# dell-research-harvard/effocr

Hardware: AMD Instinct MI355X
Metric: glyph-crops/sec end-to-end (encode+kNN), 224x224 bs=1024 (higher is better)
Workload: dtype bf16; 1 GPU; BASELINE configs[1]: vit_small_patch16_224 encoder (bf16 MFMA operands, fp32 accumulate/residual/LN/softmax), 1024x3x224x224 fp32 crops per GPU resident in HBM, 10000-row fp32 IndexFlatIP, k=10; seeded random-init weights; crops_per_gpu=1024, global_batch=1024, index_rows=10000, k=10, parallelism=1024 crops per GPU, weights+index replicated

## Files before the change

effocr_amd/_lib.py:

```python
import ctypes
import os
import subprocess
import threading

_HERE = os.path.dirname(os.path.abspath(__file__))
_CSRC = os.path.join(_HERE, "csrc")
SO_PATH = os.environ.get("EFFOCR_HIP_LIB") or os.path.join(_HERE, "libeffocr_hip.so")
SO_PATH_AB = os.path.join(_HERE, "libeffocr_hip_ab.so")

ABI_VERSION = 9
PREC = {"bf16": 0, "fp16": 1, "fp32": 2}
EPI = {"bias": 0, "bias_gelu": 1, "bias_resid": 2}

_lock = threading.Lock()
_lib = None
_loaded = {}


class EffOCRHipError(RuntimeError):
    pass


def build(force=False, verbose=False, ab=True):
    so = os.path.join(_HERE, "libeffocr_hip.so")
# ... 16 lines not shown
        SO_PATH = path or os.environ.get("EFFOCR_HIP_LIB") or os.path.join(_HERE, "libeffocr_hip.so")
        if SO_PATH != prev:
            _lib = _loaded.get(SO_PATH)
            if _lib is not None:
                EXPORTS = sorted(_declare(_lib).keys())
    return prev


def _declare(lib):
    c = ctypes
    vp, i32, i64, sz, f32p, i64p = c.c_void_p, c.c_int, c.c_int64, c.c_size_t, c.c_void_p, c.c_void_p
    sig = {
        "effocr_abi_version": (i32, []),
        "effocr_last_error": (c.c_char_p, []),
        "effocr_encoder_create": (i32, [c.c_char_p, i32, i32, c.POINTER(vp)]),
        "effocr_encoder_destroy": (None, [vp]),
        "effocr_encoder_embed_dim": (i32, [vp]),
        "effocr_encoder_num_params": (i32, [vp]),
        "effocr_encoder_param_name": (c.c_char_p, [vp, i32]),
        "effocr_encoder_param_numel": (i64, [vp, i32]),
        "effocr_encoder_set_param": (i32, [vp, c.c_char_p, vp, i64]),
        "effocr_encoder_weights_bytes": (sz, [vp]),
        "effocr_encoder_upload": (i32, [vp, vp, sz]),
        "effocr_encoder_workspace_bytes": (sz, [vp, i32]),
        "effocr_encoder_forward": (i32, [vp, f32p, i32, f32p, i32, vp, sz, vp]),
        "effocr_encoder_forward_ex": (i32, [vp, vp, i32, i32, f32p, i32, vp, sz, vp]),
        "effocr_encoder_check_status": (i32, [vp, vp, vp]),
        "effocr_encoder_reset_status": (i32, [vp, vp, vp]),
        "effocr_clock_sample": (i32, [vp, vp]),
        "effocr_encoder_set_chunk": (i32, [vp, i32]),
        "effocr_encoder_set_option": (i32, [vp, c.c_char_p, i32]),
        "effocr_op_ln_linear": (i32, [i32, i32, f32p, f32p, f32p, c.c_float, vp, f32p, f32p, vp, i32, i32, i32, vp]),
        "effocr_encoder_profile_begin": (i32, [vp, i32, c.c_char_p]),
        "effocr_encoder_profile_collect": (i32, [vp]),
        "effocr_encoder_profile_get": (i32, [vp, i32, c.POINTER(c.c_char_p), c.POINTER(c.c_double), c.POINTER(i32),
                                             c.POINTER(c.c_double)]),
        "effocr_encoder_profile_clock": (i32, [vp, i32, c.POINTER(c.c_double)]),
        "effocr_knn_workspace_bytes": (sz, [i64, i64, i32, i32]),
        "effocr_knn_ip_topk": (i32, [f32p, i64, f32p, i64, i32, i32, f32p, i64p, vp, sz, vp]),
        "effocr_knn_screen_workspace_bytes": (sz, [i64, i64, i32, i32]),
        "effocr_knn_set_option": (i32, [c.c_char_p, i32]),
        "effocr_knn_screen_flag_offset": (sz, [i64, i64, i32, i32]),
        "effocr_knn_ip_topk_screened": (i32, [f32p, i64, f32p, vp, i64, i32, i32, c.c_float, f32p, i64p, vp, sz, vp]),
        "effocr_convert_bf16": (i32, [f32p, i64, vp, vp]),
        "effocr_bf16_blocked_bytes": (sz, [i64, i32]),
        "effocr_convert_bf16_blocked": (i32, [f32p, i64, i32, vp, vp]),
        "effocr_knn_ip_topk_screened2": (i32, [f32p, i64, f32p, vp, vp, i64, i32, i32, c.c_float, f32p, i64p, vp, sz, vp]),
        "effocr_l2_normalize": (i32, [f32p, i64, i32, f32p, vp]),
        "effocr_gather_rows": (i32, [f32p, i64p, i64, i32, f32p, vp]),
        "effocr_crop_transform": (i32, [vp, i32, i32, i64, vp, i32, i32, i32, c.POINTER(c.c_float), c.POINTER(c.c_float),
                                        c.POINTER(c.c_float), f32p, vp]),
        "effocr_crop_transform_batch": (i32, [vp, i32, i64, i32, i32, i64, vp, i64, i32, i32, c.POINTER(c.c_float), c.POINTER(c.c_float),
                                              c.POINTER(c.c_float), f32p, vp]),
        "effocr_crop_transform_batch_ex": (i32, [vp, i32, i64, i32, i32, i64, vp, i64, i32, i32, c.POINTER(c.c_float), c.POINTER(c.c_float),
                                                 c.POINTER(c.c_float), i32, vp, vp]),
        "effocr_localizer_create": (i32, [c.c_char_p, i32, i32, i32, c.POINTER(vp)]),
        "effocr_localizer_destroy": (None, [vp]),
        "effocr_localizer_num_params": (i32, [vp]),
        "effocr_localizer_param_name": (c.c_char_p, [vp, i32]),
        "effocr_localizer_param_numel": (i64, [vp, i32]),
        "effocr_localizer_set_param": (i32, [vp, c.c_char_p, vp, i64]),
        "effocr_localizer_weights_bytes": (sz, [vp]),
        "effocr_localizer_upload": (i32, [vp, vp, sz]),
        "effocr_localizer_set_option": (i32, [vp, c.c_char_p, i32]),
        "effocr_localizer_num_predictions": (i64, [vp]),
        "effocr_localizer_num_outputs": (i32, [vp]),
        "effocr_localizer_workspace_bytes": (sz, [vp, i32]),
        "effocr_localizer_forward": (i32, [vp, f32p, i32, f32p, vp, sz, vp]),
        "effocr_letterbox": (i32, [vp, i32, i32, i64, i32, i32, i32, i32, i32, i32, i32, f32p, vp]),
        "effocr_nms_workspace_bytes": (sz, [i32, i32]),
        "effocr_nms_batch_workspace_bytes": (sz, [i32, i32, i32]),
        "effocr_nms": (i32, [f32p, i32, i32, c.c_float, c.c_float, i32, i32, c.c_float, i32, f32p, vp, vp, sz, vp]),
        "effocr_nms_batch": (i32, [f32p, i32, i32, i32, c.c_float, c.c_float, i32, i32, c.c_float, i32, f32p, vp, vp, sz, vp]),
        "effocr_parse_char_boxes": (i32, [f32p, vp, i32, i32, i32, i32, i32, i32, f32p, vp, vp, vp, vp]),
        "effocr_op_linear": (i32, [i32, i32, vp, vp, f32p, f32p, vp, i32, i32, i32, vp]),
        "effocr_op_layernorm": (i32, [i32, f32p, i64, i32, f32p, f32p, c.c_float, vp, vp]),
        "effocr_op_attention": (i32, [i32, vp, vp, i32, i32, i32, vp]),
        "effocr_op_linear_blocked": (i32, [i32, i32, vp, vp, f32p, f32p, vp, i32, i32, i32, i32, vp]),
        "effocr_op_mlp_blocked": (i32, [i32, f32p, f32p, f32p, c.c_float, vp, f32p, vp, f32p, f32p, i32, i32, i32, i32, vp, sz, vp]),
        "effocr_op_mlp_ln_blocked": (i32, [i32, f32p, f32p, f32p, c.c_float, vp, f32p, vp, f32p, f32p, f32p, f32p, vp, i32, i32, i32, i32, vp, sz, vp]),
        "effocr_op_proj_mlp_blocked": (i32, [i32, f32p, vp, vp, f32p, f32p, f32p, c.c_float, vp, f32p, vp, f32p, f32p, i32, i32, i32, i32, vp, sz, vp]),
        "effocr_op_qkv_attn_blocked": (i32, [i32, vp, vp, f32p, vp, i32, i32, i32, i32, vp]),
        "effocr_op_layernorm_blocked": (i32, [i32, f32p, i64, i32, f32p, f32p, c.c_float, vp, vp]),
    }
    for name, (res, args) in sig.items():
        if os.environ.get("EFFOCR_HIP_LIB") and not hasattr(lib, name):
            def _absent(*a, _n=name, **k):
                raise EffOCRHipError(f"{_n} is not exported by the library EFFOCR_HIP_LIB points at")
            setattr(lib, name, _absent)
            continue
        fn = getattr(lib, name)
        fn.restype = res
        fn.argtypes = args
    return sig


EXPORTS = None


def lib():
    global _lib, EXPORTS
    with _lock:
        if _lib is None:
            if not os.path.exists(SO_PATH):
                raise EffOCRHipError(
                    f"{SO_PATH} not found: the HIP extension is required (no CPU fallback). "
                    "Run `python -c 'import __graft_entry__ as g; g.build()'` or `make -C effocr_amd/csrc`.")
            handle = ctypes.CDLL(SO_PATH)
            EXPORTS = sorted(_declare(handle).keys())
            got = handle.effocr_abi_version()
            older_ok = bool(os.environ.get("EFFOCR_HIP_LIB")) and os.environ.get("EFFOCR_HIP_ALLOW_OLDER_ABI") == "1" and 0 < got <= ABI_VERSION
            if got != ABI_VERSION and not older_ok:
                raise EffOCRHipError(f"libeffocr_hip.so ABI version {got} != {ABI_VERSION} expected by this package: rebuild (make -C effocr_amd/csrc)")
            _lib = _loaded[SO_PATH] = handle
    return _lib


_family = {}


def _load_family(so_path, prefix, abi_version, signatures, label):
    with _lock:
        handle = _family.get(prefix)
        if handle is None:
            if not os.path.exists(so_path):
                raise EffOCRHipError(f"{so_path} not found: the {label} library is required (no CPU fallback). "
                                     "Run `python -c 'import __graft_entry__ as g; g.build()'` or `make -C effocr_amd/csrc`.")
            handle = ctypes.CDLL(so_path)
            for name, (res, args) in signatures.items():
                fn = getattr(handle, name)
                fn.restype, fn.argtypes = res, args
            got = getattr(handle, f"effocr_{prefix}_abi_version")()
            if got != abi_version:
                raise EffOCRHipError(f"{os.path.basename(so_path)} ABI version {got} != {abi_version} expected by this package: rebuild "
                                     "(make -C effocr_amd/csrc)")
            _family[prefix] = handle
    return handle


def _family_check(prefix):
    def check(rc, what=""):
        if rc != 0:
            msg = getattr(globals()[f"{prefix}_lib"](), f"effocr_{prefix}_last_error")()
            raise EffOCRHipError(f"{what} failed (code {rc}): {msg.decode() if msg else '?'}")
    check.__name__ = f"{prefix}_check"
    return check


HEAD_SO_PATH = os.path.join(_HERE, "libeffocr_head.so")
HEAD_ABI_VERSION = 1
HEAD_EXPORTS = ("effocr_head_abi_version", "effocr_head_last_error", "effocr_classifier_head_workspace_bytes",
                "effocr_classifier_head")


def _head_signatures():
    c = ctypes
    return {
        "effocr_head_abi_version": (c.c_int, []),
        "effocr_head_last_error": (c.c_char_p, []),
        "effocr_classifier_head_workspace_bytes": (c.c_size_t, [c.c_int64, c.c_int]),
        "effocr_classifier_head": (c.c_int, [c.c_void_p, c.c_int64, c.c_int, c.c_void_p, c.c_void_p, c.c_int, c.c_void_p,
                                             c.c_void_p, c.c_void_p, c.c_size_t, c.c_void_p]),
    }


def head_lib():
# ... 336 lines not shown
```

effocr_amd/csrc/api.hip:

```cpp
#include "../../include/effocr_hip.h"
#include "enc_core.hpp"


#include <math.h>
#include <algorithm>
#include <string.h>
#include <map>
#include <memory>
#include <string>
#include <vector>

namespace effocr {

namespace {

struct Param { std::string name; std::vector<int64_t> shape; int64_t numel; std::vector<float> data; bool set; };

struct VitCfg { int D, depth, heads, mlp; };
struct VitLayerOff { size_t ln1w, ln1b, qkvb, projb, ln2w, ln2b, fc1b, fc2b, qkvw, projw, fc1w, fc2w;
                     size_t qkvw_b, projw_b, fc1w_b, fc2w_b, projw_pp, fc2w_pp, projb_p, fc2b_p, qkvw_bv, qkvb_v;
                     size_t qkvw_bf, qkv_s, qkv_c, fc1w_bf, fc1_s, fc1_c; };
struct ConvSpec { std::string w, bn; int cin, cout, k, stride, pad; size_t w_off, b_off; };
struct CnxBlockOff { size_t dww, dwb, lnw, lnb, w1, b1, w2, b2, gamma; };
struct CnxStageOff { int C, Cp, depth; size_t dslnw, dslnb, dsw, dsb; std::vector<CnxBlockOff> blocks; };

}
}

using namespace effocr;

struct effocr_encoder {
  std::string arch;
  bool is_vit = false;
  int img = 224, prec = PREC_BF16, D = 0;
  std::vector<Param> params;
  std::map<std::string, int> index;
  VitCfg vit{};
  int T = 0, P = 0;
  size_t off_clspos0 = 0, off_pos = 0, off_patchb = 0, off_normw = 0, off_normb = 0, off_patchw = 0, off_patchw_b = 0;
  std::vector<VitLayerOff> layers;
  std::vector<ConvSpec> convs;
  bool is_cnx = false;
  std::vector<CnxStageOff> cnx;
  size_t cnx_stemw = 0, cnx_stemb = 0, cnx_stemlnw = 0, cnx_stemlnb = 0, cnx_headw = 0, cnx_headb = 0;
  bool is_mnv = false;
  MnvNet mnv{};
  size_t wbytes = 0;
  const char* wdev = nullptr;
  int debug = 0;
  int cls_only_last = 1;
  int mlp_stagger_min_rounds = 2;
  int mlp_tail_first = 96;
  int mlp_stagger = 2500;
  int use_projf = 1;
  int use_qkvattn = 1;
  int qa_min_batch = 1;
  int qa_hsplit = 0;
  int use_patchf = 1;
  int use_mlp = 1;
  int use_gemm3 = 1;
  int use_lnfold = 1;
  int tail_split = 1;
  int split6 = 1;
  int pair_parts = 1;
  int mlp_pair = 0;
  int use_blocked = 1;
  int use_gemm2 = 1;
  int panel_rows = 128;
  int use_panel = 1;
  int chunk = 0;
  int call_size_invariant = 0;
  int prof_mode = 0;
  std::string prof_only;
  std::vector<std::pair<hipEvent_t, hipEvent_t>> prof_pool;
  std::vector<std::pair<int, int>> prof_rec;
  std::vector<std::string> prof_names;
  size_t prof_used = 0;
  std::vector<float> prof_ms;
  std::vector<int> prof_cnt;
  std::vector<double> prof_work;
  unsigned long long* prof_clk = nullptr;
  std::vector<double> prof_ghz;
  static constexpr size_t PROF_CLK_SLOTS = 256;
};

namespace effocr {
namespace {

int64_t prod(const std::vector<int64_t>& s) { int64_t p = 1; for (auto v : s) p *= v; return p; }

void add_param(effocr_encoder* e, const std::string& name, std::vector<int64_t> shape) {
  Param p; p.name = name; p.shape = shape; p.numel = prod(shape); p.set = false;
  e->index[name] = (int)e->params.size();
  e->params.push_back(std::move(p));
}

void build_vit(effocr_encoder* e) {
  const int D = e->vit.D, depth = e->vit.depth, mlp = e->vit.mlp;
  e->P = (e->img / 16) * (e->img / 16);
  e->T = e->P + 1;
  add_param(e, "cls_token", {1, 1, D});
  add_param(e, "pos_embed", {1, e->T, D});
  add_param(e, "patch_embed.proj.weight", {D, 3, 16, 16});
  add_param(e, "patch_embed.proj.bias", {D});
  for (int i = 0; i < depth; ++i) {
    const std::string p = "blocks." + std::to_string(i) + ".";
    add_param(e, p + "norm1.weight", {D});
    add_param(e, p + "norm1.bias", {D});
    add_param(e, p + "attn.qkv.weight", {3 * D, D});
    add_param(e, p + "attn.qkv.bias", {3 * D});
    add_param(e, p + "attn.proj.weight", {D, D});
    add_param(e, p + "attn.proj.bias", {D});
    add_param(e, p + "norm2.weight", {D});
    add_param(e, p + "norm2.bias", {D});
    add_param(e, p + "mlp.fc1.weight", {mlp, D});
    add_param(e, p + "mlp.fc1.bias", {mlp});
    add_param(e, p + "mlp.fc2.weight", {D, mlp});
    add_param(e, p + "mlp.fc2.bias", {D});
  }
  add_param(e, "norm.weight", {D});
  add_param(e, "norm.bias", {D});

  const size_t es = prec_esize(e->prec);
  Alloc a;
  e->off_clspos0 = a.take((size_t)D * 4);
  e->off_pos = a.take((size_t)e->T * D * 4);
  e->off_patchb = a.take((size_t)D * 4);
  e->layers.resize(depth);
  for (int i = 0; i < depth; ++i) {
    VitLayerOff& L = e->layers[i];
    L.ln1w = a.take((size_t)D * 4); L.ln1b = a.take((size_t)D * 4);
    L.qkvb = a.take((size_t)3 * D * 4); L.projb = a.take((size_t)D * 4);
    L.ln2w = a.take((size_t)D * 4); L.ln2b = a.take((size_t)D * 4);
// ... 396 lines not shown
      put_pw(b.pwl, p + ".conv_pwl.weight", p + ".bn3");
    }
    if (r.se) { put_plain(b.ser, p + ".se.conv_reduce"); put_plain(b.see, p + ".se.conv_expand"); }
  }
  put_pw(n.cn, "blocks.5.0.conv.weight", "blocks.5.0.bn1");
  const auto& hw = P(e, "conv_head.weight"); const auto& hb = P(e, "conv_head.bias");
  put_op(blob, n.head.w, hw.data(), hw.size(), e->prec); put_f32(blob, n.head.b, hb.data(), hb.size());
}

int prof_class(effocr_encoder* e, const char* name) {
  for (size_t i = 0; i < e->prof_names.size(); ++i) if (e->prof_names[i] == name) return (int)i;
  e->prof_names.push_back(name);
  e->prof_work.push_back(0.0);
  return (int)e->prof_names.size() - 1;
}

template <typename F>
int timed(effocr_encoder* e, const char* name, double work, hipStream_t s, F launch) {
  const bool on = e->prof_mode == 1 || (e->prof_mode == 2 && e->prof_only == name);
  if (!on) return launch();
  if (e->prof_used == e->prof_pool.size()) {
    hipEvent_t a, b;
    if (hipEventCreate(&a) != hipSuccess || hipEventCreate(&b) != hipSuccess) return fail(EFFOCR_EHIP, "profile: hipEventCreate failed");
    e->prof_pool.push_back({a, b});
  }
  const int cls = prof_class(e, name);
  const size_t slot = e->prof_used++;
  const bool clk = e->prof_mode == 1 && slot < effocr_encoder::PROF_CLK_SLOTS &&
                   (e->prof_clk || hipMalloc(&e->prof_clk, effocr_encoder::PROF_CLK_SLOTS * 8192 * sizeof(unsigned long long)) == hipSuccess && hipMemset(e->prof_clk, 0, effocr_encoder::PROF_CLK_SLOTS * 8192 * sizeof(unsigned long long)) == hipSuccess);
  if (clk) (void)clock_sample(e->prof_clk + slot * 8192, s);
  (void)hipEventRecord(e->prof_pool[slot].first, s);
  const int rc = launch();
  (void)hipEventRecord(e->prof_pool[slot].second, s);
  if (clk) (void)clock_sample(e->prof_clk + slot * 8192 + 4096, s);
  e->prof_rec.push_back({cls, (int)slot});
  e->prof_work[cls] += work;
  return rc;
}

struct VitWs { size_t status, x, xn, qkv, att, h, stats, total, rows, hbytes; };
VitWs vit_ws(const effocr_encoder* e, int B) {
  const size_t M = align_up((size_t)B * e->T, 128), D = e->vit.D, es = prec_esize(e->prec);
  Alloc a; VitWs w;
  w.rows = M;
  w.status = a.take(256);
  w.x = a.take(M * D * 4);
  w.xn = a.take(M * D * es);
  w.qkv = a.take(M * 3 * D * es);
  w.att = a.take(M * D * es);
  size_t hb = M * e->vit.mlp * es, pb = (size_t)B * e->P * 768 * es;
  w.hbytes = hb > pb ? hb : pb;
  {
    const size_t cus = (size_t)device_cus(), np = M / 128, tail = np % cus;
    const size_t split = (tail && tail * 6 <= cus) ? 6 : (tail && tail * 4 <= cus) ? 4 : (tail && tail * 2 <= cus) ? 2 : 0;
    const size_t need = split * tail * 128 * D * 4;
    if (need > w.hbytes) w.hbytes = need;
  }
  w.h = a.take(w.hbytes);
  w.stats = a.take(M * 64);
  w.total = a.off;
  return w;
}

int vit_forward(effocr_encoder* e, const void* x, int x16, int B, float* emb, int l2, char* ws, hipStream_t s) {
  const VitWs w = vit_ws(e, B);
  const int D = e->vit.D, T = e->T, Pn = e->P, M = B * T, prec = e->prec;
  const char* wb = e->wdev;
  float* xs = reinterpret_cast<float*>(ws + w.x);
  void* xn = ws + w.xn; void* qkv = ws + w.qkv; void* att = ws + w.att; void* hb = ws + w.h;
  auto F = [&](size_t off) { return reinterpret_cast<const float*>(wb + off); };
  int rc;
  const double Md = (double)M, Dd = (double)D, Hd = (double)e->vit.mlp;
  const bool panel = e->use_panel && panel_gemm_supported(prec, 3 * D, D) && panel_gemm_supported(prec, e->vit.mlp, D);
  const bool g2 = e->use_gemm2 && gemm2_supported(prec, D, e->vit.mlp);
  const bool g2p = e->use_gemm2 && gemm2_supported(prec, D, 768);
  const bool g3all = !panel && e->use_gemm3 && gemm3_supported(prec, 3 * D, D) && gemm3_supported(prec, D, D) &&
                     gemm3_supported(prec, e->vit.mlp, D) && gemm3_supported(prec, D, e->vit.mlp);
  const int blk = (e->use_blocked && g2p && ((panel && g2) || g3all)) ? 1 : 0;
  const bool mlpf = blk && panel && e->use_mlp && mlp_fused_supported(prec, D, e->vit.mlp);
  const bool projf = mlpf && e->use_projf;
  const bool qaf = blk && panel && mlpf && qkv_attn_supported(prec, D, T) && (e->use_qkvattn == 2 || (e->use_qkvattn == 1 && (e->call_size_invariant || B >= e->qa_min_batch)));
  const bool g3 = blk && e->use_gemm3 && gemm3_supported(prec, D, e->vit.mlp);
  const bool patchf = blk && e->use_patchf && patch_embed_fused_supported(prec, D);
  if (!patchf && (rc = timed(e, "im2col_patch16", 0.0, s, [&] { return im2col_patch16(prec, x, x16, B, e->img, e->img, hb, s); }))) return rc;
  int* status = reinterpret_cast<int*>(ws + w.status);
  if (!patchf && (rc = set_cls_rows(F(e->off_clspos0), xs, B, T, D, blk, nullptr, s))) return rc;
  GemmArgs g{};
  if (patchf) {
    PatchArgs pa{};
    pa.x = x; pa.x16 = x16; pa.B = B; pa.H = e->img; pa.W = e->img; pa.Wb = wb + e->off_patchw_b; pa.bias = F(e->off_patchb); pa.pos = F(e->off_pos);
    pa.out = xs; pa.D = D; pa.P = Pn; pa.cls = F(e->off_clspos0);
    if ((rc = timed(e, "patch_embed_fused", 2.0 * B * Pn * Dd * 768.0, s, [&] { return patch_embed_fused(prec, pa, s); }))) return rc;
  } else {
  g.X = hb; g.ldx = 768; g.W = wb + e->off_patchw; g.ldw = 768; g.bias = F(e->off_patchb);
  g.out = xs; g.ldo = D; g.pos = F(e->off_pos); g.M = B * Pn; g.N = D; g.K = 768; g.P = Pn; g.blk_out = blk;
  if ((rc = timed(e, "gemm_patch_embed", 2.0 * B * Pn * Dd * 768.0, s, [&] { return g2p ? gemm2_nt(prec, EPI_PATCH, g, s) : gemm_nt(prec, EPI_PATCH, g, s); }))) return rc;
  }
  const float* cls_x = nullptr;
  bool xn_ready = false;
  for (int i = 0; i < e->vit.depth; ++i) {
    const VitLayerOff& L = e->layers[i];
    if (panel) {
      {
      PanelArgs p{};
      if (qaf) {
        if (!xn_ready && (rc = timed(e, "layernorm", 0.0, s, [&] { return layernorm_rows_blocked(prec, xs, M, D, F(L.ln1w), F(L.ln1b), 1e-6f, xn, s); }))) return rc;
        xn_ready = false;
        QkvAttnArgs q{};
        q.xn = xn; q.Wb = wb + L.qkvw_bv; q.bias = F(L.qkvb_v); q.out = att;
        q.B = B; q.T = T; q.D = D; q.rows_alloc = (int64_t)w.rows; q.hsplit = e->qa_hsplit;
        q.cls_only = (i + 1 == e->vit.depth && e->cls_only_last && projf) ? 1 : 0;
        const bool cls_k = q.cls_only && D == 384 && T > 192;
        const double qa_work = cls_k ? 2.0 * Md * 2.0 * Dd * Dd + 2.0 * (32.0 * B) * Dd * Dd + 4.0 * B * e->vit.heads * 32.0 * T * 64.0
                                     : 2.0 * Md * 3.0 * Dd * Dd + 4.0 * B * e->vit.heads * (double)T * T * 64.0;
        if ((rc = timed(e, "qkv_attn_fused", qa_work, s, [&] { return qkv_attn_fused(prec, q, s); }))) return rc;
      } else {
      p.A = xs; p.lda = D; p.gamma = F(L.ln1w); p.beta = F(L.ln1b); p.eps = 1e-6f; p.W = wb + L.qkvw; p.bias = F(L.qkvb);
      p.out = qkv; p.ldo = 3 * D; p.M = M; p.N = 3 * D; p.K = D; p.rows_padded = 1; p.debug = e->debug; p.panel_rows = e->panel_rows; p.no_tail_split = !e->tail_split;
      p.blk_a = blk; p.blk_out = blk;
      if ((rc = timed(e, "panel_ln_qkv", 2.0 * Md * 3.0 * Dd * Dd, s, [&] { return panel_gemm(prec, PRO_LN, EPI_BIAS, p, s); }))) return rc;
      if ((rc = timed(e, "attention", 4.0 * B * e->vit.heads * (double)T * T * 64.0, s, [&] { return attention(prec, qkv, att, B, T, e->vit.heads, blk, s); }))) return rc;
      }
      if (!projf) {
      p = PanelArgs{};
      p.A = att; p.lda = D; p.W = wb + L.projw; p.bias = F(L.projb); p.out = xs; p.ldo = D; p.resid = xs; p.ldr = D;
      p.M = M; p.N = D; p.K = D; p.rows_padded = 1; p.debug = e->debug; p.panel_rows = e->panel_rows; p.no_tail_split = !e->tail_split; p.blk_a = blk; p.blk_out = blk;
      if ((rc = timed(e, "panel_proj_resid", 2.0 * Md * Dd * Dd, s, [&] { return panel_gemm(prec, PRO_COPY, EPI_BIAS_RESID, p, s); }))) return rc;
      }
      }
      if (mlpf) {
        MlpArgs m{};
        m.x = xs; m.gamma = F(L.ln2w); m.beta = F(L.ln2b); m.eps = 1e-6f; m.W1b = wb + L.fc1w_b; m.b1 = F(L.fc1b);
        m.W2p = wb + L.fc2w_pp; m.b2 = F(L.fc2b_p); m.b2_logical = F(L.fc2b); m.M = M; m.D = D; m.H = e->vit.mlp; m.rows_alloc = (int)w.rows;
        m.partial = reinterpret_cast<float*>(hb); m.partial_bytes = w.hbytes; m.no_tail_split = !e->tail_split; m.no_split6 = !e->split6; m.pair = e->mlp_pair; m.no_pair_parts = !e->pair_parts; m.stagger = e->mlp_stagger; m.stagger_min_rounds = e->mlp_stagger_min_rounds; m.tail_first = e->mlp_tail_first;
        if (e->call_size_invariant) { m.no_tail_split = 1; m.pair = -1; }
        if (projf) {
          m.A = att; m.Wpp = wb + L.projw_pp; m.bp = F(L.projb_p);
          if (i + 1 == e->vit.depth && e->cls_only_last) {
            const size_t Bp = align_up((size_t)B, 128);
            float* xc = reinterpret_cast<float*>(qkv);
            void* ac = static_cast<char*>(qkv) + Bp * D * 4;
            if ((rc = timed(e, "gather_cls", 0.0, s, [&] { return gather_cls_rows_blocked(xs, att, B, T, D, xc, ac, s); }))) return rc;
            m.x = xc; m.A = ac; m.M = B; m.rows_alloc = (int)Bp;
            const double Bd = B;
            if ((rc = timed(e, "proj_mlp_cls", 4.0 * Bd * Hd * Dd + 2.0 * Bd * Dd * Dd, s, [&] { return mlp_fused(prec, m, s); }))) return rc;
            cls_x = xc;
            continue;
          }
          if (qaf && i + 1 < e->vit.depth) {
            m.xn_out = xn; m.gamma_n = F(e->layers[i + 1].ln1w); m.beta_n = F(e->layers[i + 1].ln1b);
            xn_ready = true;
          }
          if ((rc = timed(e, "proj_mlp_fused", 4.0 * Md * Hd * Dd + 2.0 * Md * Dd * Dd, s, [&] { return mlp_fused(prec, m, s); }))) return rc;
          continue;
        }
        if (qaf && i + 1 < e->vit.depth) {
          m.xn_out = xn; m.gamma_n = F(e->layers[i + 1].ln1w); m.beta_n = F(e->layers[i + 1].ln1b);
          xn_ready = true;
        }
        if ((rc = timed(e, "mlp_fused", 4.0 * Md * Hd * Dd, s, [&] { return mlp_fused(prec, m, s); }))) return rc;
        continue;
      }
      PanelArgs p{};
      p.A = xs; p.lda = D; p.gamma = F(L.ln2w); p.beta = F(L.ln2b); p.eps = 1e-6f; p.W = wb + L.fc1w; p.bias = F(L.fc1b);
      p.out = hb; p.ldo = e->vit.mlp; p.M = M; p.N = e->vit.mlp; p.K = D; p.rows_padded = 1; p.debug = e->debug; p.panel_rows = e->panel_rows; p.no_tail_split = !e->tail_split;
      p.blk_a = blk; p.blk_out = blk;
      if ((rc = timed(e, "panel_ln_fc1_gelu", 2.0 * Md * Hd * Dd, s, [&] { return panel_gemm(prec, PRO_LN, EPI_BIAS_GELU, p, s); }))) return rc;
    } else if (blk) {
      const bool fold = e->use_lnfold && g3 && gemm3_lnfold_supported(D);
      float* stats = reinterpret_cast<float*>(ws + w.stats);
      auto lin = [&](const void* X, int K, size_t wblk, const float* bias, void* out, int N, int epi, int fl = 0, const float* cs = nullptr) {
        GemmArgs q{};
        q.X = X; q.ldx = K; q.Wblk = wb + wblk; q.bias = bias; q.out = out; q.ldo = N; q.M = M; q.N = N; q.K = K;
        q.blk_x = 1; q.blk_out = 1; q.rows_alloc = (int)w.rows; q.no_tail_split = !e->tail_split;
        if (epi == EPI_BIAS_RESID) { q.resid = xs; q.ldr = N; }
        if (fl == 1) { q.lnf = 1; q.lnf_stats = stats; q.lnf_s = cs; q.lnf_eps = 1e-6f; }
        if (fl == 2) { q.stats = stats; q.x16 = xn; }
        return gemm3_nt(prec, epi, q, s);
      };
      const bool fold1 = fold && i > 0;
      if (!fold1 && (rc = timed(e, "layernorm", 0.0, s, [&] { return layernorm_rows_blocked(prec, xs, M, D, F(L.ln1w), F(L.ln1b), 1e-6f, xn, s); }))) return rc;
      if ((rc = timed(e, "gemm_qkv", 2.0 * Md * 3.0 * Dd * Dd, s, [&] {
            return fold1 ? lin(xn, D, L.qkvw_bf, F(L.qkv_c), qkv, 3 * D, EPI_BIAS, 1, F(L.qkv_s)) : lin(xn, D, L.qkvw_b, F(L.qkvb), qkv, 3 * D, EPI_BIAS); }))) return rc;
      if ((rc = timed(e, "attention", 4.0 * B * e->vit.heads * (double)T * T * 64.0, s, [&] { return attention(prec, qkv, att, B, T, e->vit.heads, 1, s); }))) return rc;
      const size_t Bp = align_up((size_t)B, 256);
      if (i + 1 == e->vit.depth && e->cls_only_last && g3 && Bp <= w.rows) {
        float* xc = reinterpret_cast<float*>(qkv);
        void* ac = static_cast<char*>(qkv) + Bp * D * 4;
        if ((rc = timed(e, "gather_cls", 0.0, s, [&] { return gather_cls_rows_blocked(xs, att, B, T, D, xc, ac, s); }))) return rc;
        auto linc = [&](const void* X, int K, size_t wblk, const float* bias, void* out, int N, int epi, int fl = 0, const float* cs = nullptr) {
          GemmArgs q{};
          q.X = X; q.ldx = K; q.Wblk = wb + wblk; q.bias = bias; q.out = out; q.ldo = N; q.M = B; q.N = N; q.K = K;
          q.blk_x = 1; q.blk_out = 1; q.rows_alloc = (int)Bp; q.no_tail_split = !e->tail_split;
          if (epi == EPI_BIAS_RESID) { q.resid = xc; q.ldr = N; }
          if (fl == 1) { q.lnf = 1; q.lnf_stats = stats; q.lnf_s = cs; q.lnf_eps = 1e-6f; }
          if (fl == 2) { q.stats = stats; q.x16 = xn; }
          return gemm3_nt(prec, epi, q, s);
        };
        const double Bd = B;
        if ((rc = timed(e, "cls_proj_resid", 2.0 * Bd * Dd * Dd, s, [&] { return linc(ac, D, L.projw_b, F(L.projb), xc, D, EPI_BIAS_RESID, fold ? 2 : 0); }))) return rc;
        if (!fold && (rc = timed(e, "layernorm", 0.0, s, [&] { return layernorm_rows_blocked(prec, xc, B, D, F(L.ln2w), F(L.ln2b), 1e-6f, xn, s); }))) return rc;
        if ((rc = timed(e, "cls_fc1_gelu", 2.0 * Bd * Hd * Dd, s, [&] {
              return fold ? linc(xn, D, L.fc1w_bf, F(L.fc1_c), hb, e->vit.mlp, EPI_BIAS_GELU, 1, F(L.fc1_s)) : linc(xn, D, L.fc1w_b, F(L.fc1b), hb, e->vit.mlp, EPI_BIAS_GELU); }))) return rc;
        if ((rc = timed(e, "cls_fc2_resid", 2.0 * Bd * Dd * Hd, s, [&] { return linc(hb, e->vit.mlp, L.fc2w_b, F(L.fc2b), xc, D, EPI_BIAS_RESID); }))) return rc;
        cls_x = xc;
        continue;
      }
      if ((rc = timed(e, "gemm_proj_resid", 2.0 * Md * Dd * Dd, s, [&] { return lin(att, D, L.projw_b, F(L.projb), xs, D, EPI_BIAS_RESID, fold ? 2 : 0); }))) return rc;
      if (!fold && (rc = timed(e, "layernorm", 0.0, s, [&] { return layernorm_rows_blocked(prec, xs, M, D, F(L.ln2w), F(L.ln2b), 1e-6f, xn, s); }))) return rc;
      if ((rc = timed(e, "gemm_fc1_gelu", 2.0 * Md * Hd * Dd, s, [&] {
            return fold ? lin(xn, D, L.fc1w_bf, F(L.fc1_c), hb, e->vit.mlp, EPI_BIAS_GELU, 1, F(L.fc1_s)) : lin(xn, D, L.fc1w_b, F(L.fc1b), hb, e->vit.mlp, EPI_BIAS_GELU); }))) return rc;
      if (fold && g3 && i + 1 < e->vit.depth) {
        GemmArgs q{};
        q.X = hb; q.ldx = e->vit.mlp; q.Wblk = wb + L.fc2w_b; q.bias = F(L.fc2b); q.out = xs; q.ldo = D; q.resid = xs; q.ldr = D;
        q.M = M; q.N = D; q.K = e->vit.mlp; q.blk_x = 1; q.blk_out = 1; q.rows_alloc = (int)w.rows; q.no_tail_split = !e->tail_split;
        q.stats = stats; q.x16 = xn;
        if ((rc = timed(e, "gemm_fc2_resid", 2.0 * Md * Dd * Hd, s, [&] { return gemm3_nt(prec, EPI_BIAS_RESID, q, s); }))) return rc;
        continue;
      }
    } else {
      if ((rc = timed(e, "layernorm", 0.0, s, [&] { return layernorm_rows(prec, xs, M, D, F(L.ln1w), F(L.ln1b), 1e-6f, xn, s); }))) return rc;
      g = GemmArgs{};
      g.X = xn; g.ldx = D; g.W = wb + L.qkvw; g.ldw = D; g.bias = F(L.qkvb); g.out = qkv; g.ldo = 3 * D;
      g.M = M; g.N = 3 * D; g.K = D;
      if ((rc = timed(e, "gemm_qkv", 2.0 * Md * 3.0 * Dd * Dd, s, [&] { return gemm_nt(prec, EPI_BIAS, g, s); }))) return rc;
      if ((rc = timed(e, "attention", 4.0 * B * e->vit.heads * (double)T * T * 64.0, s, [&] { return attention(prec, qkv, att, B, T, e->vit.heads, 0, s); }))) return rc;
      g = GemmArgs{};
      g.X = att; g.ldx = D; g.W = wb + L.projw; g.ldw = D; g.bias = F(L.projb); g.out = xs; g.ldo = D;
      g.resid = xs; g.ldr = D; g.M = M; g.N = D; g.K = D;
      if ((rc = timed(e, "gemm_proj_resid", 2.0 * Md * Dd * Dd, s, [&] { return gemm_nt(prec, EPI_BIAS_RESID, g, s); }))) return rc;
      if ((rc = timed(e, "layernorm", 0.0, s, [&] { return layernorm_rows(prec, xs, M, D, F(L.ln2w), F(L.ln2b), 1e-6f, xn, s); }))) return rc;
      g = GemmArgs{};
      g.X = xn; g.ldx = D; g.W = wb + L.fc1w; g.ldw = D; g.bias = F(L.fc1b); g.out = hb; g.ldo = e->vit.mlp;
      g.M = M; g.N = e->vit.mlp; g.K = D;
// ... 245 lines not shown
    if (!(T <= 64 || (T > 192 && T <= 224)))
      return fail(EFFOCR_EUNSUPPORTED, "vit: token count must be <= 64 or in (192, 224] (img_size 224)");
    e->is_vit = true; e->D = e->vit.D;
    build_vit(e.get());
  }
  *out = e.release();
  return EFFOCR_OK;
}

void effocr_encoder_destroy(effocr_encoder_t* enc) {
  if (!enc) return;
  for (auto& ev : enc->prof_pool) { (void)hipEventDestroy(ev.first); (void)hipEventDestroy(ev.second); }
  if (enc->prof_clk) (void)hipFree(enc->prof_clk);
  delete enc;
}
int effocr_encoder_embed_dim(const effocr_encoder_t* enc) { return enc ? enc->D : 0; }
int effocr_encoder_num_params(const effocr_encoder_t* enc) { return enc ? (int)enc->params.size() : 0; }
const char* effocr_encoder_param_name(const effocr_encoder_t* enc, int i) {
  if (!enc || i < 0 || i >= (int)enc->params.size()) return nullptr;
  return enc->params[i].name.c_str();
}
int64_t effocr_encoder_param_numel(const effocr_encoder_t* enc, int i) {
  if (!enc || i < 0 || i >= (int)enc->params.size()) return -1;
  return enc->params[i].numel;
}

int effocr_encoder_set_param(effocr_encoder_t* enc, const char* name, const float* host, int64_t numel) {
  if (!enc || !name || !host) return fail(EFFOCR_EINVAL, "set_param: NULL argument");
  auto it = enc->index.find(name);
  if (it == enc->index.end()) return fail(EFFOCR_EINVAL, std::string("set_param: unknown parameter '") + name + "'");
  Param& p = enc->params[it->second];
  if (p.numel != numel)
    return fail(EFFOCR_EINVAL, std::string("set_param: '") + name + "' expects " + std::to_string(p.numel) +
                                   " elements, got " + std::to_string(numel));
  p.data.assign(host, host + numel);
  p.set = true;
  return EFFOCR_OK;
}

size_t effocr_encoder_weights_bytes(const effocr_encoder_t* enc) { return enc ? enc->wbytes : 0; }

int effocr_encoder_upload(effocr_encoder_t* enc, void* weights_dev, size_t bytes) {
  if (!enc || !weights_dev) return fail(EFFOCR_EINVAL, "upload: NULL argument");
  if (bytes < enc->wbytes) return fail(EFFOCR_EWORKSPACE, "upload: weight buffer too small");
  for (const Param& p : enc->params)
    if (!p.set) return fail(EFFOCR_ESTATE, "upload: parameter '" + p.name + "' was never set");
  std::vector<char> blob(enc->wbytes, 0);
  if (enc->is_vit) pack_vit(enc, blob); else if (enc->is_cnx) pack_convnext(enc, blob); else if (enc->is_mnv) pack_mobilenetv3(enc, blob);
  else pack_resnet(enc, blob);
  const hipError_t er = hipMemcpy(weights_dev, blob.data(), enc->wbytes, hipMemcpyHostToDevice);
  if (er != hipSuccess) return fail(EFFOCR_EHIP, std::string("upload: hipMemcpy: ") + hipGetErrorString(er));
  enc->wdev = static_cast<const char*>(weights_dev);
  return EFFOCR_OK;
}

size_t effocr_encoder_workspace_bytes(const effocr_encoder_t* enc, int batch) {
  if (!enc || batch <= 0) return 0;
  if (enc->is_cnx) return convnext_ws(enc, cnx_chunk(enc, batch)).total;
  if (enc->is_mnv) return mnv3_ws(enc, mnv3_chunk(enc, batch)).total;
  if (!enc->is_vit) return resnet_ws(enc, batch).total;
  return vit_ws(enc, (enc->chunk > 0 && enc->chunk < batch) ? enc->chunk : batch).total;
}

int effocr_encoder_set_option(effocr_encoder_t* enc, const char* name, int value) {
  if (!enc || !name) return fail(EFFOCR_EINVAL, "set_option: NULL argument");
  const std::string n = name;
  if (n == "use_panel") { enc->use_panel = value; return EFFOCR_OK; }
  if (n == "debug") { enc->debug = value; return EFFOCR_OK; }
  if (n == "use_gemm2") { enc->use_gemm2 = value; return EFFOCR_OK; }
  if (n == "use_blocked") { enc->use_blocked = value; return EFFOCR_OK; }
  if (n == "tail_split") { enc->tail_split = value; return EFFOCR_OK; }
  if (n == "split6") { enc->split6 = value; return EFFOCR_OK; }
  if (n == "mlp_pair") { enc->mlp_pair = value; return EFFOCR_OK; }
  if (n == "pair_parts") { enc->pair_parts = value; return EFFOCR_OK; }
  if (n == "use_gemm3") { enc->use_gemm3 = value; return EFFOCR_OK; }
  if (n == "use_lnfold") { enc->use_lnfold = value; return EFFOCR_OK; }
  if (n == "use_mlp") { enc->use_mlp = value; return EFFOCR_OK; }
  if (n == "use_qkvattn") { enc->use_qkvattn = value; return EFFOCR_OK; }
  if (n == "qa_min_batch") { enc->qa_min_batch = value; return EFFOCR_OK; }
  if (n == "qa_hsplit") { enc->qa_hsplit = value; return EFFOCR_OK; }
  if (n == "use_patchf") { enc->use_patchf = value; return EFFOCR_OK; }
  if (n == "use_projf") { enc->use_projf = value; return EFFOCR_OK; }
  if (n == "cls_only_last") { enc->cls_only_last = value; return EFFOCR_OK; }
  if (n == "mlp_stagger_min_rounds") { enc->mlp_stagger_min_rounds = value < 1 ? 1 : value; return EFFOCR_OK; }
  if (n == "mlp_tail_first") { enc->mlp_tail_first = value < 0 ? 0 : value & ~7; return EFFOCR_OK; }
  if (n == "mlp_stagger") { enc->mlp_stagger = value < 0 ? 0 : value; return EFFOCR_OK; }
  if (n == "panel_rows") { if (value != 64 && value != 128) return fail(EFFOCR_EINVAL, "set_option: panel_rows must be 64 or 128"); enc->panel_rows = value; return EFFOCR_OK; }
  if (n == "call_size_invariant") {
    if (value != 0 && value != 1) return fail(EFFOCR_EINVAL, "set_option: call_size_invariant must be 0 or 1");
    enc->call_size_invariant = value; return EFFOCR_OK;
  }
  if (n == "chunk") { if (value < 0) return fail(EFFOCR_EINVAL, "set_option: chunk < 0"); enc->chunk = value; return EFFOCR_OK; }
  return fail(EFFOCR_EINVAL, "set_option: unknown option '" + n + "'");
}

int effocr_encoder_set_chunk(effocr_encoder_t* enc, int crops_per_chunk) {
  if (!enc || crops_per_chunk < 0) return fail(EFFOCR_EINVAL, "set_chunk: bad argument");
  enc->chunk = crops_per_chunk;
  return EFFOCR_OK;
}

int effocr_encoder_forward(effocr_encoder_t* enc, const float* x_dev, int batch, float* emb_dev, int l2_normalize,
                           void* workspace_dev, size_t workspace_bytes, void* stream) {
  return effocr_encoder_forward_ex(enc, x_dev, EFFOCR_PREC_FP32, batch, emb_dev, l2_normalize, workspace_dev, workspace_bytes, stream);
}

int effocr_encoder_forward_ex(effocr_encoder_t* enc, const void* x_dev, int x_dtype, int batch, float* emb_dev, int l2_normalize,
                              void* workspace_dev, size_t workspace_bytes, void* stream) {
  if (!enc) return fail(EFFOCR_EINVAL, "forward: NULL encoder");
  if (x_dtype != PREC_FP32 && !(enc->is_vit && enc->prec != PREC_FP32 && x_dtype == enc->prec))
    return fail(x_dtype < 0 || x_dtype > 2 ? EFFOCR_EINVAL : EFFOCR_EUNSUPPORTED,
                "forward: crops must be fp32, or (ViT, 16-bit precision modes) already in the encoder's own operand type");
  const int x16 = x_dtype != PREC_FP32;
  if (batch < 0) return fail(EFFOCR_EINVAL, "forward: negative batch");
  if (batch == 0) return EFFOCR_OK;
  if (!x_dev || !emb_dev || !workspace_dev) return fail(EFFOCR_EINVAL, "forward: NULL device pointer");
  if (!enc->wdev) return fail(EFFOCR_ESTATE, "forward: weights were not uploaded");
  if (workspace_bytes < effocr_encoder_workspace_bytes(enc, batch)) return fail(EFFOCR_EWORKSPACE, "forward: workspace too small");
  if ((int64_t)batch * (enc->is_vit ? enc->T : enc->img * enc->img) >= (int64_t)1 << 30)
    return fail(EFFOCR_EUNSUPPORTED, "forward: batch too large for 32-bit row indices");
  char* ws = static_cast<char*>(workspace_dev);
  if (enc->is_cnx) {
    const int chunk = cnx_chunk(enc, batch);
    const int64_t so = enc->img / 4;
    if ((int64_t)chunk * so * so * 4 * enc->cnx[0].C >= (int64_t)1 << 31)
      return fail(EFFOCR_EUNSUPPORTED, "forward: chunk too large for 32-bit GEMM row indices (effocr_encoder_set_chunk)");
    const size_t img_bytes = (size_t)3 * enc->img * enc->img * 4;
    for (int b0 = 0; b0 < batch; b0 += chunk) {
      const int cb = (batch - b0 < chunk) ? batch - b0 : chunk;
      const int rc = convnext_forward(enc, reinterpret_cast<const float*>(static_cast<const char*>(x_dev) + (size_t)b0 * img_bytes), cb,
                                      emb_dev + (size_t)b0 * enc->D, l2_normalize, ws, S(stream));
      if (rc) return rc;
    }
    return EFFOCR_OK;
  }
  if (enc->is_mnv) {
    const int chunk = mnv3_chunk(enc, batch);
    const size_t img_bytes = (size_t)3 * enc->img * enc->img * 4;
    for (int b0 = 0; b0 < batch; b0 += chunk) {
      const int cb = (batch - b0 < chunk) ? batch - b0 : chunk;
      const int rc = mnv3_forward(enc, reinterpret_cast<const float*>(static_cast<const char*>(x_dev) + (size_t)b0 * img_bytes), cb,
                                  emb_dev + (size_t)b0 * enc->D, l2_normalize, ws, S(stream));
      if (rc) return rc;
    }
    return EFFOCR_OK;
  }
  if (!enc->is_vit) return resnet_forward(enc, static_cast<const float*>(x_dev), batch, emb_dev, l2_normalize, ws, S(stream));
  const int chunk = enc->chunk > 0 ? enc->chunk : batch;
  const size_t img_bytes = (size_t)3 * enc->img * enc->img * (x16 ? 2 : 4);
  for (int b0 = 0; b0 < batch; b0 += chunk) {
    const int cb = (batch - b0 < chunk) ? batch - b0 : chunk;
    const int rc = vit_forward(enc, static_cast<const char*>(x_dev) + (size_t)b0 * img_bytes, x16, cb, emb_dev + (size_t)b0 * enc->D, l2_normalize, ws, S(stream));
    if (rc) return rc;
  }
  return EFFOCR_OK;
}

int effocr_clock_sample(void* out_dev, void* stream) {
  if (!out_dev) return fail(EFFOCR_EINVAL, "clock_sample: NULL pointer");
  return clock_sample(static_cast<unsigned long long*>(out_dev), S(stream));
}

int effocr_encoder_check_status(const effocr_encoder_t* enc, const void* workspace_dev, void* stream) {
  if (!enc || !workspace_dev) return fail(EFFOCR_EINVAL, "check_status: NULL argument");
  if (!enc->is_vit && !enc->is_cnx && !enc->is_mnv) return EFFOCR_OK;
  int st = 0;
// ... 187 lines not shown
    p.A = x_dev; p.lda = k; p.W = w_dev; p.bias = bias_dev; p.out = out_dev; p.ldo = n; p.resid = resid_dev; p.ldr = n;
    p.M = m; p.N = n; p.K = k;
    return panel_gemm(precision, PRO_COPY, epilogue, p, S(stream));
  }
  GemmArgs g{};
  g.X = x_dev; g.ldx = k; g.W = w_dev; g.ldw = k; g.bias = bias_dev; g.out = out_dev; g.ldo = n;
  g.resid = resid_dev; g.ldr = n; g.M = m; g.N = n; g.K = k;
  if (gemm2_supported(precision, n, k)) return gemm2_nt(precision, epilogue, g, S(stream));
  return gemm_nt(precision, epilogue, g, S(stream));
}

int effocr_op_ln_linear(int precision, int epilogue, const float* x_dev, const float* gamma_dev, const float* beta_dev,
                        float eps, const void* w_dev, const float* bias_dev, const float* resid_dev, void* out_dev,
                        int m, int n, int k, void* stream) {
  if (epilogue < 0 || epilogue > 2) return fail(EFFOCR_EINVAL, "op_ln_linear: unknown epilogue");
  PanelArgs p{};
  p.A = x_dev; p.lda = k; p.gamma = gamma_dev; p.beta = beta_dev; p.eps = eps; p.W = w_dev; p.bias = bias_dev;
  p.out = out_dev; p.ldo = n; p.resid = resid_dev; p.ldr = n; p.M = m; p.N = n; p.K = k;
  return panel_gemm(precision, PRO_LN, epilogue, p, S(stream));
}


int effocr_op_linear_blocked(int precision, int epilogue, const void* x_blk_dev, const void* w_blk_dev, const float* bias_dev,
                             const float* resid_blk_dev, void* out_blk_dev, int m, int n, int k, int rows_alloc, void* stream) {
  if (epilogue < 0 || epilogue > 2) return fail(EFFOCR_EINVAL, "op_linear_blocked: unknown epilogue");
  if (m > 0 && (!x_blk_dev || !w_blk_dev || !bias_dev || !out_blk_dev || (epilogue == EPI_BIAS_RESID && !resid_blk_dev)))
    return fail(EFFOCR_EINVAL, "op_linear_blocked: NULL device pointer");
  GemmArgs g{};
  g.X = x_blk_dev; g.ldx = k; g.Wblk = w_blk_dev; g.bias = bias_dev; g.out = out_blk_dev; g.ldo = n;
  g.resid = resid_blk_dev; g.ldr = n; g.M = m; g.N = n; g.K = k; g.blk_x = 1; g.blk_out = 1; g.rows_alloc = rows_alloc;
  return gemm3_nt(precision, epilogue, g, S(stream));
}

int effocr_op_mlp_blocked(int precision, float* x_blk_dev, const float* gamma_dev, const float* beta_dev, float eps,
                          const void* w1_blk_dev, const float* b1_dev, const void* w2_perm_dev, const float* b2_perm_dev, const float* b2_dev,
                          int m, int d, int h, int rows_alloc, void* scratch_dev, size_t scratch_bytes, void* stream) {
  if (m > 0 && (!x_blk_dev || !gamma_dev || !beta_dev || !w1_blk_dev || !b1_dev || !w2_perm_dev || !b2_perm_dev || !b2_dev))
    return fail(EFFOCR_EINVAL, "op_mlp_blocked: NULL device pointer");
  MlpArgs a{};
  a.x = x_blk_dev; a.gamma = gamma_dev; a.beta = beta_dev; a.eps = eps; a.W1b = w1_blk_dev; a.b1 = b1_dev; a.W2p = w2_perm_dev; a.b2 = b2_perm_dev;
  a.b2_logical = b2_dev;
  a.M = m; a.D = d; a.H = h; a.rows_alloc = rows_alloc; a.partial = static_cast<float*>(scratch_dev); a.partial_bytes = scratch_bytes;
  return mlp_fused(precision, a, S(stream));
}

int effocr_op_mlp_ln_blocked(int precision, float* x_blk_dev, const float* gamma_dev, const float* beta_dev, float eps,
                             const void* w1_blk_dev, const float* b1_dev, const void* w2_perm_dev, const float* b2_perm_dev, const float* b2_dev,
                             const float* gamma_next_dev, const float* beta_next_dev, void* xn_blk_dev,
                             int m, int d, int h, int rows_alloc, void* scratch_dev, size_t scratch_bytes, void* stream) {
  if (m > 0 && (!x_blk_dev || !gamma_dev || !beta_dev || !w1_blk_dev || !b1_dev || !w2_perm_dev || !b2_perm_dev || !b2_dev || !gamma_next_dev || !beta_next_dev || !xn_blk_dev))
    return fail(EFFOCR_EINVAL, "op_mlp_ln_blocked: NULL device pointer");
  MlpArgs a{};
  a.x = x_blk_dev; a.gamma = gamma_dev; a.beta = beta_dev; a.eps = eps; a.W1b = w1_blk_dev; a.b1 = b1_dev; a.W2p = w2_perm_dev; a.b2 = b2_perm_dev;
  a.b2_logical = b2_dev;
  a.M = m; a.D = d; a.H = h; a.rows_alloc = rows_alloc; a.partial = static_cast<float*>(scratch_dev); a.partial_bytes = scratch_bytes;
  a.xn_out = xn_blk_dev; a.gamma_n = gamma_next_dev; a.beta_n = beta_next_dev;
  return mlp_fused(precision, a, S(stream));
}

int effocr_op_proj_mlp_blocked(int precision, float* x_blk_dev, const void* a_blk_dev, const void* wp_perm_dev, const float* bp_perm_dev,
                               const float* gamma_dev, const float* beta_dev, float eps, const void* w1_blk_dev, const float* b1_dev,
                               const void* w2_perm_dev, const float* b2_perm_dev, const float* b2_dev, int m, int d, int h, int rows_alloc,
                               void* scratch_dev, size_t scratch_bytes, void* stream) {
  if (m > 0 && (!x_blk_dev || !a_blk_dev || !wp_perm_dev || !bp_perm_dev || !gamma_dev || !beta_dev || !w1_blk_dev || !b1_dev || !w2_perm_dev || !b2_perm_dev || !b2_dev))
    return fail(EFFOCR_EINVAL, "op_proj_mlp_blocked: NULL device pointer");
  MlpArgs a{};
  a.x = x_blk_dev; a.gamma = gamma_dev; a.beta = beta_dev; a.eps = eps; a.W1b = w1_blk_dev; a.b1 = b1_dev; a.W2p = w2_perm_dev; a.b2 = b2_perm_dev;
  a.b2_logical = b2_dev; a.A = a_blk_dev; a.Wpp = wp_perm_dev; a.bp = bp_perm_dev;
  a.M = m; a.D = d; a.H = h; a.rows_alloc = rows_alloc; a.partial = static_cast<float*>(scratch_dev); a.partial_bytes = scratch_bytes;
  return mlp_fused(precision, a, S(stream));
}

int effocr_op_qkv_attn_blocked(int precision, const void* xn_blk_dev, const void* wqkv_blk_dev, const float* bias_dev,
                               void* out_blk_dev, int batch, int tokens, int d, int rows_alloc, void* stream) {
  if (batch > 0 && (!xn_blk_dev || !wqkv_blk_dev || !bias_dev || !out_blk_dev))
    return fail(EFFOCR_EINVAL, "op_qkv_attn_blocked: NULL device pointer");
  if (batch < 0 || tokens < 1) return fail(EFFOCR_EINVAL, "op_qkv_attn_blocked: bad batch / tokens");
  QkvAttnArgs q{};
  q.xn = xn_blk_dev; q.Wb = wqkv_blk_dev; q.bias = bias_dev; q.out = out_blk_dev;
  q.B = batch; q.T = tokens; q.D = d; q.rows_alloc = rows_alloc;
  return qkv_attn_fused(precision, q, S(stream));
}

int effocr_op_layernorm_blocked(int out_precision, const float* x_blk_dev, int64_t rows, int d, const float* gamma_dev,
                                const float* beta_dev, float eps, void* out_blk_dev, void* stream) {
  if (rows > 0 && (!x_blk_dev || !gamma_dev || !beta_dev || !out_blk_dev)) return fail(EFFOCR_EINVAL, "op_layernorm_blocked: NULL device pointer");
  return layernorm_rows_blocked(out_precision, x_blk_dev, rows, d, gamma_dev, beta_dev, eps, out_blk_dev, S(stream));
}

int effocr_op_layernorm(int out_precision, const float* x_dev, int64_t rows, int d, const float* gamma_dev,
                        const float* beta_dev, float eps, void* out_dev, void* stream) {
  return layernorm_rows(out_precision, x_dev, rows, d, gamma_dev, beta_dev, eps, out_dev, S(stream));
}

int effocr_op_attention(int precision, const void* qkv_dev, void* out_dev, int batch, int tokens, int heads, void* stream) {
  return attention(precision, qkv_dev, out_dev, batch, tokens, heads, 0, S(stream));
}

}
```

effocr_amd/csrc/kernels.hpp:

```cpp
#pragma once
#include "common.hpp"

namespace effocr {

enum { PREC_BF16 = 0, PREC_FP16 = 1, PREC_FP32 = 2 };
enum { EPI_BIAS = 0, EPI_BIAS_GELU = 1, EPI_BIAS_RESID = 2, EPI_PATCH = 3,
       EPI_BIAS_SCALE_RESID = 4,
       EPI_BIAS_F32 = 5 };

static inline int prec_esize(int prec) { return prec == PREC_FP32 ? 4 : 2; }

struct GemmArgs {
  const void* X; int64_t ldx;
  const void* W; int64_t ldw;
  const float* bias;
  void* out; int64_t ldo;
  const float* resid; int64_t ldr;
  const float* pos;
  int M, N, K;
  int P;
  int blk_x;
  int blk_out;
  const void* Wblk;
  int rows_alloc;
  int no_tail_split;
  float* stats; void* x16;
  const float* lnf_stats; const float* lnf_s; int lnf; float lnf_eps;
  const float* scale;
};

int gemm_nt(int prec, int epi, const GemmArgs& g, hipStream_t s);

bool gemm2_supported(int prec, int N, int K);
int gemm2_nt(int prec, int epi, const GemmArgs& g, hipStream_t s);

bool gemm3_supported(int prec, int N, int K);
bool gemm3_lnfold_supported(int D);
int gemm3_nt(int prec, int epi, const GemmArgs& g, hipStream_t s);

struct MlpArgs {
  float* x;
  const float* gamma; const float* beta; float eps;
  const void* W1b; const float* b1;
  const void* W2p; const float* b2;
  int M, D, H;
  int rows_alloc;
  float* partial; size_t partial_bytes;
  int no_tail_split;
  int no_split6;
  int no_pair_parts;
  int pair;
  int panel0, tail_rb, stagger_wgs, main_wgs;
  int stagger;
  int stagger_min_rounds;
  int tail_first;
  const void* A; const void* Wpp; const float* bp; const float* b2_logical;
  void* xn_out; const float* gamma_n; const float* beta_n;
};
bool mlp_fused_supported(int prec, int D, int H);
int mlp_fused(int prec, const MlpArgs& a, hipStream_t s);

struct QkvAttnArgs {
  const void* xn;
  const void* Wb; const float* bias;
  void* out;
  int B, T, D;
  int64_t rows_alloc;
  int cls_only;
  int img0;
  int hsplit;
};
bool qkv_attn_supported(int prec, int D, int T);
int qkv_attn_fused(int prec, const QkvAttnArgs& a, hipStream_t s);

struct PatchArgs {
  const void* x; int B, H, W;
  int x16;
  const void* Wb;
  const float* bias; const float* pos;
  const float* cls;
  float* out;
  int D, P;
};
bool patch_embed_fused_supported(int prec, int D);
int patch_embed_fused(int prec, const PatchArgs& a, hipStream_t s);

enum { PRO_COPY = 0, PRO_LN = 1 };
struct PanelArgs {
  const void* A; int64_t lda;
  const float* gamma; const float* beta; float eps;
  const void* W;
  const float* bias;
  void* out; int64_t ldo;
  const float* resid; int64_t ldr;
  int M, N, K;
  unsigned long long* dbg;
  int debug;
  int blk_a;
  int blk_out;
  int panel_rows;
  int rows_padded;
  int no_tail_split;
  int tail_first, tail_split;
};
bool panel_gemm_supported(int prec, int N, int K);
int panel_gemm(int prec, int pro, int epi, const PanelArgs& a, hipStream_t s);

int reduce_layernorm_rows_blocked(int prec_out, float* x, int64_t rows, int D, const float* partial, const float* b2, int nparts, int tail_rb,
                                  int add_x, const float* gamma, const float* beta, float eps, void* out, hipStream_t s);
int layernorm_rows_blocked(int prec_out, const float* x, int64_t rows, int D, const float* gamma, const float* beta,
                           float eps, void* out, hipStream_t s);
int layernorm_rows(int prec_out, const float* x, int64_t rows, int D, const float* gamma, const float* beta,
                   float eps, void* out, hipStream_t s);
int im2col_patch16(int prec_out, const void* x, int x16, int B, int H, int W, void* out, hipStream_t s);
int clock_sample(unsigned long long* out, hipStream_t s);
int set_cls_rows(const float* cls_pos0, float* x, int B, int T, int D, int blocked, int* status_zero, hipStream_t s);
int gather_cls_rows_blocked(const float* x, const void* att, int B, int T, int D, float* xc, void* ac, hipStream_t s);
int attention(int prec, const void* qkv, void* out, int B, int T, int heads, int blocked, hipStream_t s);
int final_cls_norm(const float* x, int B, int T, int D, const float* gamma, const float* beta, float eps,
                   int l2norm, int blocked, float* emb, int* status, hipStream_t s);

size_t knn_workspace_bytes(int64_t B, int64_t N, int D, int k);
int knn_ip_topk(const float* q, int64_t B, const float* xb, int64_t N, int D, int k, float* dist, int64_t* idx,
                void* ws, size_t ws_bytes, hipStream_t s);
size_t knn_screen_workspace_bytes(int64_t B, int64_t N, int D, int k);
void knn_set_wg_target(int n);
void knn_q16_tile(int on);
void knn_two_pass_screen(int on);
void knn_force_tile_kernel(int on);
size_t knn_screen_flag_offset(int64_t B, int64_t N, int D, int k);
int knn_ip_topk_screened(const float* q, int64_t B, const float* xb, const void* xb16, const void* xblk, int64_t N, int D, int k, float xnorm_max,
                         float* dist, int64_t* idx, void* ws, size_t ws_bytes, hipStream_t s);
int convert_bf16_blocked(const float* src, int64_t N, int D, void* dst, hipStream_t s);
void knn_qs_option(int which, int value);
int convert_bf16(const float* src, int64_t n, void* dst, hipStream_t s);
int l2_normalize_rows(const float* x, int64_t B, int D, float* y, hipStream_t s);
int gather_rows(const float* src, const int64_t* rows, int64_t n, int D, float* dst, hipStream_t s);

int crop_transform(const uint8_t* img, int n_img, int64_t img_stride, int H, int W, int64_t stride, const int* boxes, int box_ld, int64_t n, int S,
                   int antialias, const float* mean, const float* stdv, const float* fill, void* out, int out_prec, hipStream_t s);

struct ConvArgs {
  const float* in;
  const float* w;
  const float* bias;
  const float* resid;
  float* out;
  int B, H, W, Cin, Cout, KH, KW, stride, pad, OH, OW, relu;
  int in_ld, in_off, out_ld, out_off, res_ld, res_off;
  int silu;
  float* partial; size_t partial_bytes;
  int ksplit;
  const void* w16;
};
int conv2d_nhwc(const ConvArgs& a, hipStream_t s);
int im2col_conv1(const float* x, float* col, int B, int H, int W, int OH, int OW, hipStream_t s);
int maxpool3x3s2_nhwc(const float* in, float* out, int B, int H, int W, int C, int OH, int OW, hipStream_t s);
int global_avgpool_nhwc(const float* in, float* out, int B, int HW, int C, int l2norm, hipStream_t s);

int im2col_nchw(const float* x, float* col, int B, int Cin, int H, int W, int KH, int KW, int stride, int pad, int OH, int OW, int kpad, hipStream_t s);
int stem6x6s2_nchw(const float* x, const float* w, int w_ld, const float* wt, const float* bias, float* out, int B, int H, int W, int OH, int OW, int out_ld,
                   int out_off, int silu, hipStream_t s);
int stem6x6s2_g16_nchw(const float* x, const float* wt, int wt_ld, const float* bias, float* out, int B, int H, int W, int OH, int OW, int out_ld,
                       int out_off, int cout, int cout_st, hipStream_t s);
int upsample2x_nhwc(const float* in, int in_ld, int in_off, float* out, int out_ld, int out_off, int B, int H, int W, int C, hipStream_t s);
int maxpool5_nhwc(const float* in, int in_ld, int in_off, float* out, int out_ld, int out_off, int B, int H, int W, int C, hipStream_t s);
int yolo_decode(const float* raw, int raw_ld, float* pred, int B, int ny, int nx, int na, int no, float stride, const float* anchors_px,
                int64_t total, int64_t row0, hipStream_t s);
int letterbox_u8(const uint8_t* img, int H, int W, int64_t row_stride, int bgr, int out_h, int out_w, int new_h, int new_w, int top, int left,
                 float fill, float* out, hipStream_t s);
size_t nms_workspace_bytes(int n, int max_nms);
bool nms_greedy_applies(int n, int max_det, int max_nms);
int nms_yolo_batch(const float* pred, int B, int n, int nc, float conf_thres, float iou_thres, int max_det, int max_nms, float max_wh, int agnostic,
                   float* out, int* count, void* ws, size_t ws_bytes, hipStream_t s);
int nms_yolo(const float* pred, int n, int nc, float conf_thres, float iou_thres, int max_det, int max_nms, float max_wh, int agnostic,
             float* out, int* count, void* ws, size_t ws_bytes, hipStream_t s);

int stem3x3s2_nchw(const float* x, const float* wt, int wt_ld, const float* bias, float* out, int B, int H, int W, int OH, int OW, int out_ld, int out_off,
                   int cout, int cout_st, hipStream_t s);
int yolov8_decode(const float* box, int box_ld, const float* cls, int cls_ld, float* pred, int B, int ny, int nx, int nc, float stride, int64_t total,
                  int64_t row0, hipStream_t s);

constexpr int Y11_MAX_TOKENS = 1600;
int attention_nhwc(const float* qkv, int qkv_ld, int qkv_off, float* out, int out_ld, int out_off, int B, int N, int heads, hipStream_t s);
int dwconv3x3_nhwc(const float* in, int in_ld, int in_off, int icut, int istride, const float* w, const float* bias, int silu, const float* add, int add_ld,
                   int add_off, float* out, int out_ld, int out_off, int B, int H, int W, int C, hipStream_t s);

int cnx_stem(const float* img, int B, int S, const float* wt, const float* bias, const float* lnw, const float* lnb, int C0, float* x, hipStream_t s);
int cnx_dwconv_ln(int prec, const float* x, int B, int H, int W, int C, int Cp, const float* w, const float* bias, const float* lnw,
                  const float* lnb, void* out, hipStream_t s);
int cnx_ln_s2d(int prec, const float* x, int B, int H, int W, int C, int Cp, const float* lnw, const float* lnb, void* out, hipStream_t s);
int cnx_head(const float* x, int B, int HW, int C, int Cp, const float* lnw, const float* lnb, int l2norm, float* emb, int* status, hipStream_t s);

struct MnvConv { uint32_t w, b; };
struct MnvBlock { int cin, mid, cout, k, stride, se, hs, res, cg; MnvConv pw, dw, ser, see, pwl; };
constexpr int MNV_NBLK = 11;
struct MnvNet { int S, stem_c, cn_c, nf; MnvConv stem, cn, head; MnvBlock blk[MNV_NBLK]; };
constexpr int MNV_T1 = 8, MNV_T2 = 8;
constexpr int MNV_TAIL_LDS_FLOATS = 39680;
__host__ __device__ static inline int mnv3_tiles1(int S) { const int n = (S / 4 + MNV_T1 - 1) / MNV_T1; return n * n; }
__host__ __device__ static inline int mnv3_tiles2(int S) { const int n = (S / 8 + MNV_T2 - 1) / MNV_T2; return n * n; }
int mnv3_stem_ds(int prec, const float* img, int B, const char* wb, const MnvNet& net, float* t0, float* part, hipStream_t s);
int mnv3_stage1(int prec, const float* t0, const float* part, int B, const char* wb, const MnvNet& net, float* t1, hipStream_t s);
// ... 5 lines not shown
```

effocr_amd/csrc/mlp.hip:

```cpp
#include "common.hpp"
#include "kernels.hpp"

namespace effocr {

int mlp_launch_bf16(const MlpArgs& a, hipStream_t s);
int mlp_launch_bf16p(const MlpArgs& a, hipStream_t s);
int mlp_launch_f16(const MlpArgs& a, hipStream_t s);
int mlp_launch_f16p(const MlpArgs& a, hipStream_t s);

bool panel_gemm_supported(int prec, int N, int K) {
  return (prec == PREC_BF16 || prec == PREC_FP16) && (K == 384 || K == 128) && N > 0 && N % 128 == 0 && N <= 4 * K;
}

bool mlp_fused_supported(int prec, int D, int H) {
  return (prec == PREC_BF16 || prec == PREC_FP16) && ((D == 384 && H == 1536) || (D == 128 && H == 512));
}

int mlp_fused(int prec, const MlpArgs& a, hipStream_t s) {
  if (a.M <= 0) return EFFOCR_OK;
  if (!mlp_fused_supported(prec, a.D, a.H)) return fail(EFFOCR_EUNSUPPORTED, "mlp_fused: needs bf16/fp16 and (D, H) in {(384, 1536), (128, 512)}");
  if (a.rows_alloc % 32 != 0 || a.rows_alloc < a.M) return fail(EFFOCR_EINVAL, "mlp_fused: rows_alloc must be a multiple of 32 covering M");
  const bool proj = a.A != nullptr;
  if (proj && (!a.Wpp || !a.bp)) return fail(EFFOCR_EINVAL, "mlp_fused: the projection needs its weight and bias");
  if (!a.b2_logical) return fail(EFFOCR_EINVAL, "mlp_fused: the unpermuted fc2 bias is required");
  if (a.xn_out && (!a.gamma_n || !a.beta_n)) return fail(EFFOCR_EINVAL, "mlp_fused: the second output needs the next norm's weight and bias");
  if (prec == PREC_BF16) return proj ? mlp_launch_bf16p(a, s) : mlp_launch_bf16(a, s);
  return proj ? mlp_launch_f16p(a, s) : mlp_launch_f16(a, s);
}

}
```

effocr_amd/csrc/mlp_bf16pair.hip:

```cpp
#include "mlp_kernel.hpp"
namespace effocr {
int mlp_pair_launch_bf16(const MlpArgs& a, int tncw, unsigned grid, hipStream_t s) { return launch_mlp_pair<__bf16>(a, tncw, grid, s); }
}
#ifdef MLP_STAMP
extern "C" int effocr_debug_mlp_pair_stamps(unsigned long long* out, int n) {
  hipDeviceSynchronize();
  return (int)hipMemcpyFromSymbol(out, HIP_SYMBOL(effocr::mlp_stamps), (size_t)n * sizeof(unsigned long long));
}
#endif
```

effocr_amd/csrc/mlp_kernel.hpp:

```cpp
#pragma once
#include "common.hpp"
#include "kernels.hpp"
#include "mlp_roles.hpp"
#include <type_traits>

#ifndef MLP_BARRIER_DRAIN
#define MLP_BARRIER_DRAIN 0
#endif
#ifndef MLP_FUSED_REDUCE_LN
#define MLP_FUSED_REDUCE_LN 1
#endif
#ifndef MLP_ROWS_LATE
#define MLP_ROWS_LATE 1
#endif
#ifndef MLP_M0_ONCE
#define MLP_M0_ONCE 1
#endif
#ifndef MLP_GELU_BURST
#define MLP_GELU_BURST 2
#endif
#ifndef MLP_DIAG
#define MLP_DIAG 0
#endif
#ifndef MLP_LN_PK
// ... 847 lines not shown
    float sm = 0.f;
    sfor<0, OT>([&](auto T_) {
      constexpr int t = decltype(T_)::value;
      if constexpr (((t & 3) >> 1) == PP) {
#pragma unroll
        for (int q = 0; q < 4; ++q) {
          const f32x4 v = *reinterpret_cast<const f32x4*>(px + (t * 4 + q) * 1024);
#pragma unroll
          for (int e = 0; e < 4; ++e) acc2[t][4 * q + e] += v[e];
          const f32x4 o = {acc2[t][4 * q], acc2[t][4 * q + 1], acc2[t][4 * q + 2], acc2[t][4 * q + 3]};
          sm += (o[0] + o[1]) + (o[2] + o[3]);
          if constexpr (PARTIAL) *reinterpret_cast<f32x4*>(pr + (size_t)cq(t, q) * 512) = o;
          else if (live) st_act<4>(reinterpret_cast<f32x4*>(xr + (size_t)cq(t, q) * 512), o);
        }
      }
    });
    MLP_STAMP_AT(9)
    if (!PARTIAL && a.xn_out) {
      float* sS = reinterpret_cast<float*>(smem + 2 * (OT * 4 * 1024));
      sm += __shfl_xor(sm, 32, 64);
      if (half == 0) sS[w * 32 + r31] = sm;
      asm volatile("s_waitcnt lgkmcnt(0)" ::: "memory");
      __builtin_amdgcn_s_barrier();
      asm volatile("" ::: "memory");
      sm += sS[(w ^ 1) * 32 + r31];
      const float mean = sm * (1.0f / D);
      f32x2 q2 = {0.f, 0.f};
      const f32x2 nm = {-mean, -mean};
      sfor<0, OT>([&](auto T_) {
        constexpr int t = decltype(T_)::value;
        if constexpr (((t & 3) >> 1) == PP) {
#pragma unroll
          for (int r = 0; r < 16; r += 2) {
            const f32x2 d = f32x2{acc2[t][r], acc2[t][r + 1]} + nm;
            q2 = __builtin_elementwise_fma(d, d, q2);
          }
        }
      });
      float ss = q2[0] + q2[1];
      ss += __shfl_xor(ss, 32, 64);
      if (half == 0) sS[128 + w * 32 + r31] = ss;
      asm volatile("s_waitcnt lgkmcnt(0)" ::: "memory");
      __builtin_amdgcn_s_barrier();
      asm volatile("" ::: "memory");
      ss += sS[128 + (w ^ 1) * 32 + r31];
      const float rstd = 1.0f / sqrtf(ss * (1.0f / D) + a.eps);
      const f32x2 r2 = {rstd, rstd}, nm2 = {-mean, -mean};
      char* nr = static_cast<char*>(a.xn_out) + rb * (D / 8) * 512 + r31 * 16;
      sfor<0, OT>([&](auto T_) {
        constexpr int t = decltype(T_)::value;
        if constexpr (((t & 3) >> 1) == PP) {
#pragma unroll
          for (int p = 0; p < 2; ++p) {
            u32x2 pk[2];
#pragma unroll
            for (int j = 0; j < 2; ++j) {
              const int q = 2 * p + j, c = cq(t, q);
              const f32x4 gm = *reinterpret_cast<const f32x4*>(sGn + c * 4);
              const f32x4 bt = *reinterpret_cast<const f32x4*>(sBn + c * 4);
              const f32x2 o0 = __builtin_elementwise_fma((f32x2{acc2[t][4 * q], acc2[t][4 * q + 1]} + nm2) * r2, f32x2{gm[0], gm[1]}, f32x2{bt[0], bt[1]});
              const f32x2 o1 = __builtin_elementwise_fma((f32x2{acc2[t][4 * q + 2], acc2[t][4 * q + 3]} + nm2) * r2, f32x2{gm[2], gm[3]}, f32x2{bt[2], bt[3]});
              pk[j] = pack4<E>(o0[0], o0[1], o1[0], o1[1]);
            }
            const u32x4 o = {pk[0][0], pk[0][1], pk[1][0], pk[1][1]};
            if (live) st_act<8>(reinterpret_cast<u32x4*>(nr + (size_t)(4 * t + 2 * p + hf) * 512), o);
          }
        }
      });
    }
  }
  if constexpr (PARTIAL && !PAIR) {
    const int64_t rbl = rb - (int64_t)a.panel0 * 4;
    char* pr = reinterpret_cast<char*>(a.partial) + (((int64_t)(bid % SPLIT) * a.tail_rb + rbl) * (D / 4)) * 512 + r31 * 16;
    sfor<0, OT>([&](auto T_) {
      constexpr int t = decltype(T_)::value;
#pragma unroll
      for (int q = 0; q < 4; ++q) {
        const f32x4 o = {acc2[t][4 * q], acc2[t][4 * q + 1], acc2[t][4 * q + 2], acc2[t][4 * q + 3]};
        *reinterpret_cast<f32x4*>(pr + (size_t)cq(t, q) * 512) = o;
      }
    });
  } else if (!PAIR && !PARTIAL && rb * 32 + r31 < a.M) {
    char* xr = reinterpret_cast<char*>(a.x) + rb * (D / 4) * 512 + r31 * 16;
    float sm = 0.f;
    sfor<0, OT>([&](auto T_) {
      constexpr int t = decltype(T_)::value;
#pragma unroll
      for (int q = 0; q < 4; ++q) {
        const f32x4 o = {acc2[t][4 * q], acc2[t][4 * q + 1], acc2[t][4 * q + 2], acc2[t][4 * q + 3]};
        sm += (o[0] + o[1]) + (o[2] + o[3]);
        st_act<4>(reinterpret_cast<f32x4*>(xr + (size_t)cq(t, q) * 512), o);
      }
    });
    MLP_STAMP_AT(9)
    if (a.xn_out) {
      sm += __shfl_xor(sm, 32, 64);
      const float mean = sm * (1.0f / D);
      float ss = 0.f;
      if constexpr (MLP_LN_PK) {
        f32x2 q2 = {0.f, 0.f};
        const f32x2 nm = {-mean, -mean};
        sfor<0, OT>([&](auto T_) {
          constexpr int t = decltype(T_)::value;
#pragma unroll
          for (int r = 0; r < 16; r += 2) {
            const f32x2 d = f32x2{acc2[t][r], acc2[t][r + 1]} + nm;
            q2 = __builtin_elementwise_fma(d, d, q2);
          }
        });
        ss = q2[0] + q2[1];
      } else
      sfor<0, OT>([&](auto T_) {
        constexpr int t = decltype(T_)::value;
#pragma unroll
        for (int r = 0; r < 16; ++r) { const float d = acc2[t][r] - mean; ss += d * d; }
      });
      ss += __shfl_xor(ss, 32, 64);
      const float rstd = 1.0f / sqrtf(ss * (1.0f / D) + a.eps);
      const f32x2 r2 = {rstd, rstd}, nm2 = {-mean, -mean};
      char* nr = static_cast<char*>(a.xn_out) + rb * (D / 8) * 512 + r31 * 16;
      sfor<0, OT>([&](auto T_) {
        constexpr int t = decltype(T_)::value;
#pragma unroll
        for (int p = 0; p < 2; ++p) {
          u32x2 pk[2];
#pragma unroll
          for (int j = 0; j < 2; ++j) {
            const int q = 2 * p + j, c = cq(t, q);
            const f32x4 gm = *reinterpret_cast<const f32x4*>(sGn + c * 4);
            const f32x4 bt = *reinterpret_cast<const f32x4*>(sBn + c * 4);
            if constexpr (MLP_LN_PK) {
              const f32x2 o0 = __builtin_elementwise_fma((f32x2{acc2[t][4 * q], acc2[t][4 * q + 1]} + nm2) * r2, f32x2{gm[0], gm[1]}, f32x2{bt[0], bt[1]});
              const f32x2 o1 = __builtin_elementwise_fma((f32x2{acc2[t][4 * q + 2], acc2[t][4 * q + 3]} + nm2) * r2, f32x2{gm[2], gm[3]}, f32x2{bt[2], bt[3]});
              pk[j] = pack4<E>(o0[0], o0[1], o1[0], o1[1]);
            } else
            pk[j] = pack4<E>((acc2[t][4 * q] - mean) * rstd * gm[0] + bt[0], (acc2[t][4 * q + 1] - mean) * rstd * gm[1] + bt[1],
                             (acc2[t][4 * q + 2] - mean) * rstd * gm[2] + bt[2], (acc2[t][4 * q + 3] - mean) * rstd * gm[3] + bt[3]);
          }
          const u32x4 o = {pk[0][0], pk[0][1], pk[1][0], pk[1][1]};
          st_act<8>(reinterpret_cast<u32x4*>(nr + (size_t)(4 * t + 2 * p + hf) * 512), o);
        }
      });
    }
  }
  MLP_STAMP_AT(10)
#ifdef MLP_STAMP
  if constexpr (MLP_STAMP_ON) { mlp_stamps[MLP_STAMP_ROW + 12] = vm_wait; mlp_stamps[MLP_STAMP_ROW + 13] = bar_wait; }
  asm volatile("s_waitcnt vmcnt(0)" ::: "memory");
#endif
  MLP_STAMP_AT(11)
#ifdef MLP_STAMP
  if (MLP_STAMP_ON) mlp_stamps[MLP_STAMP_ROW + 16] = __builtin_amdgcn_s_memrealtime();
#endif
}

template <typename E, int D, int H, int TNCW, bool PROJ>
__global__ __launch_bounds__(256, 1) void mlp_fused_kernel(MlpArgs a) {
  if constexpr (TNCW == 0) {
    mlp_fused_body<E, D, H, H / 128, false, PROJ>(a, (int)blockIdx.x);
  } else {
    const MlpRole role = mlp_role_clamped((int)blockIdx.x, a.main_wgs, a.stagger_wgs, a.tail_first);
    if (!role.part) mlp_fused_body<E, D, H, H / 128, false, PROJ>(a, role.index);
    else {
      const int b = role.index;
      if constexpr (PROJ) {
        if (b % ((H / 128) / TNCW) == 0) mlp_fused_body<E, D, H, TNCW, true, true, false, true>(a, b);
        else mlp_fused_body<E, D, H, TNCW, true, true, false, false>(a, b);
      } else mlp_fused_body<E, D, H, TNCW, true, PROJ>(a, b);
    }
  }
}

template <typename E, int D, int H, int TNCW>
__global__ __launch_bounds__(256, 1) void mlp_pair_kernel(MlpArgs a) {
  const bool w1 = (wave_id() & 1) != 0;
  if constexpr (TNCW == 0) {
    if (!w1) mlp_fused_body<E, D, H, H / 128, false, true, true, true, 0>(a, (int)blockIdx.x);
    else mlp_fused_body<E, D, H, H / 128, false, true, true, true, 1>(a, (int)blockIdx.x);
  } else {
    const bool keep = (int)blockIdx.x % ((H / 128) / TNCW) == 0;
    if (keep) {
      if (!w1) mlp_fused_body<E, D, H, TNCW, true, true, true, true, 0>(a, (int)blockIdx.x);
      else mlp_fused_body<E, D, H, TNCW, true, true, true, true, 1>(a, (int)blockIdx.x);
    } else {
      if (!w1) mlp_fused_body<E, D, H, TNCW, true, true, true, false, 0>(a, (int)blockIdx.x);
      else mlp_fused_body<E, D, H, TNCW, true, true, true, false, 1>(a, (int)blockIdx.x);
    }
  }
}

__global__ __launch_bounds__(256) void mlp_reduce_kernel(float* x, const float* partial, const float* b2, int64_t rb0, int tail_rb,
                                                         int D, int nparts, int64_t M, int add_x) {
  const int64_t id = (int64_t)blockIdx.x * 256 + threadIdx.x;
  const int64_t per_rb = (int64_t)(D / 4) * 32;
  if (id >= (int64_t)tail_rb * per_rb) return;
  const int64_t rbl = id / per_rb;
  const int rem = (int)(id - rbl * per_rb), chunk = rem >> 5, row = rem & 31;
  if ((rb0 + rbl) * 32 + row >= M) return;
  f32x4* xp = reinterpret_cast<f32x4*>(x) + (rb0 + rbl) * per_rb + rem;
  f32x4 v = *xp;
  const f32x4 bv = *reinterpret_cast<const f32x4*>(b2 + chunk * 4);
  f32x4 acc = {0.f, 0.f, 0.f, 0.f};
  for (int p = 0; p < nparts; ++p) {
    const f32x4 pv = reinterpret_cast<const f32x4*>(partial)[((int64_t)p * tail_rb + rbl) * per_rb + rem];
#pragma unroll
    for (int e = 0; e < 4; ++e) acc[e] += pv[e];
  }
#pragma unroll
  for (int e = 0; e < 4; ++e) v[e] = acc[e] + bv[e] + (add_x ? v[e] : 0.f);
  *xp = v;
}

template <typename E>
int launch_mlp_pair(const MlpArgs& a, int tncw, unsigned grid, hipStream_t s) {
  switch (tncw) {
    case 0: hipLaunchKernelGGL((mlp_pair_kernel<E, 384, 1536, 0>), dim3(grid), dim3(256), 0, s, a); return check_launch("mlp_pair");
    case 2: hipLaunchKernelGGL((mlp_pair_kernel<E, 384, 1536, 2>), dim3(grid), dim3(256), 0, s, a); break;
    case 4: hipLaunchKernelGGL((mlp_pair_kernel<E, 384, 1536, 4>), dim3(grid), dim3(256), 0, s, a); break;
    case 6: hipLaunchKernelGGL((mlp_pair_kernel<E, 384, 1536, 6>), dim3(grid), dim3(256), 0, s, a); break;
    default: return fail(EFFOCR_EINVAL, "mlp_pair: hidden chunks per part must be 0 (whole), 2, 4 or 6");
  }
  return check_launch("mlp_pair_parts");
}

template <typename E, bool PROJ>
int launch_mlp(const MlpArgs& a_in, hipStream_t s) {
  MlpArgs a = a_in;
  for (const void* q : {(const void*)a.b1, (const void*)a.b2, (const void*)a.gamma, (const void*)a.beta, (const void*)a.bp, (const void*)a.gamma_n, (const void*)a.beta_n})
    if ((reinterpret_cast<uintptr_t>(q) & 15) != 0) return fail(EFFOCR_EINVAL, "mlp_fused: bias / LayerNorm parameter arrays must be 16-byte aligned (they reach LDS by 16-byte DMA)");
  const int npanels = (a.M + MLP_PT - 1) / MLP_PT;
  const int tail_first_opt = a.tail_first;
  a.tail_first = 0;
  if (a.D == 128 && a.H == 512) {
    a.panel0 = 0; a.main_wgs = npanels; a.stagger_wgs = 0;
    hipLaunchKernelGGL((mlp_fused_kernel<E, 128, 512, 0, PROJ>), dim3((unsigned)npanels), dim3(256), 0, s, a);
    return check_launch("mlp_fused");
  }
  if (!(a.D == 384 && a.H == 1536)) return fail(EFFOCR_EUNSUPPORTED, "mlp_fused: (D, H) must be (384, 1536) or (128, 512)");
  const int slots = device_cus();
  if constexpr (PROJ) {
    const int np64 = (a.M + 63) / 64;
    const bool fits = np64 <= slots && a.rows_alloc >= np64 * 64;
    const int pparts = (np64 * 6 <= slots && !a.no_split6) ? 6 : np64 * 3 <= slots ? 3 : 2;
    if (fits && (pparts > 2 || np64 * 16 <= slots * 7) && a.pair == 0 && !a.no_pair_parts && !a.no_tail_split && a.partial &&
        a.partial_bytes >= (size_t)pparts * np64 * 64 * a.D * sizeof(float)) {
      a.panel0 = 0; a.main_wgs = 0; a.stagger_wgs = 0; a.tail_rb = np64 * 2;
      const int prec = std::is_same<E, __bf16>::value ? PREC_BF16 : PREC_FP16;
      int rc = prec == PREC_BF16 ? mlp_pair_launch_bf16(a, 12 / pparts, (unsigned)(np64 * pparts), s) : mlp_pair_launch_f16(a, 12 / pparts, (unsigned)(np64 * pparts), s);
      if (rc) return rc;
      if (a.xn_out && MLP_FUSED_REDUCE_LN)
        return reduce_layernorm_rows_blocked(prec, a.x, (int64_t)a.M, a.D, a.partial, a.b2_logical, pparts, a.tail_rb, 0, a.gamma_n, a.beta_n, a.eps, a.xn_out, s);
      const int64_t slots4 = (int64_t)a.tail_rb * (a.D / 4) * 32;
      hipLaunchKernelGGL(mlp_reduce_kernel, dim3((unsigned)((slots4 + 255) / 256)), dim3(256), 0, s, a.x, a.partial, a.b2_logical, (int64_t)0, a.tail_rb, a.D, pparts, (int64_t)a.M, 0);
      rc = check_launch("mlp_reduce");
      if (rc || !a.xn_out) return rc;
      return layernorm_rows_blocked(prec, a.x, (int64_t)a.M, a.D, a.gamma_n, a.beta_n, a.eps, a.xn_out, s);
    }
    if (fits && (a.pair > 0 || (a.pair == 0 && !a.no_tail_split && npanels * 11 > slots * 2))) {
      a.panel0 = 0; a.main_wgs = np64; a.stagger_wgs = 0; a.tail_rb = 0;
      return std::is_same<E, __bf16>::value ? mlp_pair_launch_bf16(a, 0, (unsigned)np64, s) : mlp_pair_launch_f16(a, 0, (unsigned)np64, s);
    }
  }
  const int tail = a.no_tail_split ? 0 : npanels % slots;
  int split = 1;
  for (const int cand : {6, 4, 2}) {
    if (cand == 6 && a.no_split6) continue;
    if (tail > 0 && tail * cand <= slots && a.partial && a.partial_bytes >= (size_t)cand * tail * MLP_PT * a.D * sizeof(float)) { split = cand; break; }
  }
  const int main_panels = split > 1 ? npanels - tail : npanels;
  a.panel0 = main_panels;
  a.main_wgs = main_panels;
  a.tail_rb = tail * 4;
  a.stagger_wgs = main_panels >= (a.stagger_min_rounds > 0 ? a.stagger_min_rounds : 4) * slots ? slots : 0;
  a.tail_first = a.stagger > 0 ? mlp_tail_first_clamp(tail_first_opt, main_panels, tail, split, a.stagger_wgs) : 0;
  const dim3 grid((unsigned)(main_panels + (split > 1 ? tail * split : 0)));
  if (split == 6) hipLaunchKernelGGL((mlp_fused_kernel<E, 384, 1536, 2, PROJ>), grid, dim3(256), 0, s, a);
  else if (split == 4) hipLaunchKernelGGL((mlp_fused_kernel<E, 384, 1536, 3, PROJ>), grid, dim3(256), 0, s, a);
  else if (split == 2) hipLaunchKernelGGL((mlp_fused_kernel<E, 384, 1536, 6, PROJ>), grid, dim3(256), 0, s, a);
  else hipLaunchKernelGGL((mlp_fused_kernel<E, 384, 1536, 0, PROJ>), grid, dim3(256), 0, s, a);
  int rc = check_launch("mlp_fused");
  if (rc || split == 1) return rc;
  const int64_t rb0 = (int64_t)main_panels * 4;
  const int prec = std::is_same<E, __bf16>::value ? PREC_BF16 : PREC_FP16;
  if (a.xn_out && MLP_FUSED_REDUCE_LN) {
    return reduce_layernorm_rows_blocked(prec, reinterpret_cast<float*>(reinterpret_cast<char*>(a.x) + rb0 * (a.D / 4) * 512), (int64_t)a.M - rb0 * 32, a.D,
                                         a.partial, a.b2_logical, split, a.tail_rb, PROJ ? 0 : 1, a.gamma_n, a.beta_n, a.eps,
                                         static_cast<char*>(a.xn_out) + rb0 * (a.D / 8) * 512, s);
  }
  const int64_t slots4 = (int64_t)a.tail_rb * (a.D / 4) * 32;
  hipLaunchKernelGGL(mlp_reduce_kernel, dim3((unsigned)((slots4 + 255) / 256)), dim3(256), 0, s, a.x, a.partial, a.b2_logical,
                     rb0, a.tail_rb, a.D, split, (int64_t)a.M, PROJ ? 0 : 1);
  rc = check_launch("mlp_reduce");
  if (rc || !a.xn_out) return rc;
  return layernorm_rows_blocked(prec, reinterpret_cast<const float*>(reinterpret_cast<const char*>(a.x) + rb0 * (a.D / 4) * 512), (int64_t)a.M - rb0 * 32, a.D,
                                a.gamma_n, a.beta_n, a.eps, static_cast<char*>(a.xn_out) + rb0 * (a.D / 8) * 512, s);
}

}
}
```

effocr_amd/csrc/mlp_roles.hpp:

```cpp
#pragma once

namespace effocr {

struct MlpRole {
  bool part;
  int index;
};

constexpr int mlp_tail_first_clamp(int tail_first, int main_panels, int tail, int split, int slots) {
  if (tail_first <= 0 || tail <= 0 || split <= 1 || slots <= 0 || slots > 256 || slots % 8 != 0 || main_panels < slots) return 0;
  int tf = tail_first < tail * split ? tail_first : tail * split;
  if (tf > slots) tf = slots;
  return tf & ~7;
}

constexpr MlpRole mlp_role_clamped(int bid, int main_panels, int slots, int tf) {
  const int lo = slots - tf;
  const bool early = bid < lo;
  const bool first = bid < slots;
  const bool rest = bid < main_panels + tf;
  const int index = early ? bid : first ? bid - lo : rest ? bid - tf : bid - main_panels;
  return MlpRole{!(early | (rest & !first)), index};
}

constexpr MlpRole mlp_role(int bid, int main_panels, int tail, int split, int slots, int tail_first) {
  const int tf = mlp_tail_first_clamp(tail_first, main_panels, tail, split, slots);
  return mlp_role_clamped(bid, main_panels, tf > 0 ? slots : 0, tf);
}

}
```

effocr_amd/csrc/qkvattn.hip:

```cpp
#include "common.hpp"
#include "kernels.hpp"
#include <math.h>
#include <type_traits>

#ifndef QA_NT
#define QA_NT 0
#endif
#ifndef QA_ODD_TILE_WAVE
#define QA_ODD_TILE_WAVE 1
#endif
#ifndef QA_BARRIER_DRAIN
#define QA_BARRIER_DRAIN 0
#endif
#ifndef QA_EDGE_BLOCK_MAJOR
#define QA_EDGE_BLOCK_MAJOR 1
#endif

namespace effocr {
#ifdef EFFOCR_CONVOPS
thread_local int convops_qa_launches = 0, convops_qa_last[2][6] = {};
#define QA_REC(d, ntt, cls, npv) (convops_qa_launches < 2 ? (void)(convops_qa_last[convops_qa_launches][0] = (d), convops_qa_last[convops_qa_launches][1] = (ntt), \
  convops_qa_last[convops_qa_launches][2] = (cls), convops_qa_last[convops_qa_launches][3] = (npv), convops_qa_last[convops_qa_launches][4] = hs, \
  convops_qa_last[convops_qa_launches][5] = (int)grid.x) : (void)0, ++convops_qa_launches)
#else
#define QA_REC(d, ntt, cls, npv) ((void)0)
#endif
namespace {

#ifdef QA_STAMP
constexpr int QA_STAMP_WGS = 256, QA_STAMP_N = 16;
__device__ unsigned long long qa_stamps[QA_STAMP_WGS * 4 * QA_STAMP_N];
#define QA_STAMP_AT(k) qa_stamps[((blockIdx.x & (QA_STAMP_WGS - 1)) * 4 + w) * QA_STAMP_N + (k)] = __builtin_amdgcn_s_memtime();
#else
#define QA_STAMP_AT(k)
#endif

template <int I, int N, typename F> __device__ __forceinline__ void qa_for(F&& f) {
  if constexpr (I < N) {
    f(std::integral_constant<int, I>{});
    qa_for<I + 1, N>(f);
  }
}


constexpr int QA_STAGE = 16384;
constexpr int QA_RING = 6;

template <typename E, int D, int NTT, bool CLS = false, int NPV = 2 * NTT>
__global__ __launch_bounds__(256, 1) void qkvattn_kernel(QkvAttnArgs a) {
  typedef typename Op16<E>::V8 V8;
  constexpr int HEADS = D / 64;
  constexpr int KC = D / 8;
  constexpr int KT = D / 128;
  constexpr int NSH = 3 * KT;
  constexpr int NS = HEADS * NSH;
  constexpr int NXF = D / 16;
  constexpr int R = QA_RING;
  constexpr bool SMALL = NSH < R - 1;
  static_assert(D % 128 == 0 && NS >= R - 1, "qkvattn: embed dim must be a multiple of 128");
  __shared__ __attribute__((aligned(16))) char smem[R * QA_STAGE + NTT * 8192 + 3 * D * 4];
  char* sK = smem;
  char* sV = sK + NTT * 4096;
  float* sBias = reinterpret_cast<float*>(sV + NTT * 4096);
  char* sW = smem + NTT * 8192 + 3 * D * 4;

  const int tid = threadIdx.x;
  int lane = tid & 63, r31 = lane & 31, half = lane >> 5;
  auto refresh_lane = [&]() __attribute__((always_inline)) {
    asm volatile("" : "+v"(lane));
    r31 = lane & 31;
    half = lane >> 5;
  };
  const int w = wave_id();
  QA_STAMP_AT(14)
  const int T = a.T;
  int64_t tok0 = 0;
  const int HS = a.hsplit > 1 ? a.hsplit : 1, NH = HEADS / HS;
  const int grp = (int)blockIdx.x % HS, slot0 = a.img0 + (int)blockIdx.x / HS, nslots = (int)gridDim.x / HS;
  const int hb = grp * NH;
  const int h0 = ((int)blockIdx.x >> 3) % NH;
  const char* Wb = static_cast<const char*>(a.Wb);

  {
    const unsigned sB_lds = (unsigned)(size_t)(__attribute__((address_space(3))) char*)sBias;
#pragma unroll
    for (int j = 0; j < (3 * D / 4 + 255) / 256; ++j) {
      const int u = j * 256 + tid;
      const char* src = reinterpret_cast<const char*>(a.bias) + (size_t)u * 16;
      const unsigned dst = (unsigned)__builtin_amdgcn_readfirstlane((int)(sB_lds + (unsigned)(j * 256 + (tid >> 6) * 64) * 16u));
      if (u < 3 * D / 4)
        asm volatile("s_mov_b32 m0, %1\n\t"
                     "s_nop 0\n\t"
                     "global_load_lds_dwordx4 %0, off"
                     :: "v"(src), "s"(dst) : "memory", "m0");
    }
  }

  int ih = hb + h0, isec = 0, ikt = 0, islot = 0;
  const unsigned lane16 = (unsigned)(tid & 63) * 16u;
  auto issue_piece = [&](int p) __attribute__((always_inline)) {
    const int rb = (isec * D + ih * 64) / 32 + (w >> 1);
    const __attribute__((address_space(1))) void* src =
        (const __attribute__((address_space(1))) void*)(Wb + ((size_t)rb * KC + ikt * 16 + (w & 1) * 8) * 512 + lane16);
    __attribute__((address_space(3))) void* dst = (__attribute__((address_space(3))) void*)(sW + islot * QA_STAGE + ((w >> 1) * 16 + (w & 1) * 8) * 512);
    switch (p) {
      case 0: __builtin_amdgcn_global_load_lds(src, dst, 16, 0, 0); break;
      case 1: __builtin_amdgcn_global_load_lds(src, dst, 16, 1024, 0); break;
      case 2: __builtin_amdgcn_global_load_lds(src, dst, 16, 2048, 0); break;
      default: __builtin_amdgcn_global_load_lds(src, dst, 16, 3072, 0); break;
    }
  };
  const unsigned sW_lds = (unsigned)(size_t)(__attribute__((address_space(3))) char*)sW;
  auto issue_piece_asm = [&](auto P_) __attribute__((always_inline)) {
    constexpr int pc = decltype(P_)::value;
    const int rb = (isec * D + ih * 64) / 32 + (w >> 1);
    const char* src = Wb + ((size_t)rb * KC + ikt * 16 + (w & 1) * 8) * 512 + lane16;
    const unsigned dst = (unsigned)__builtin_amdgcn_readfirstlane((int)(sW_lds + (unsigned)(islot * QA_STAGE) + (unsigned)(((w >> 1) * 16 + (w & 1) * 8) * 512)));
    unsigned keep;
    asm volatile("s_mov_b32 %0, m0\n\t"
                 "s_mov_b32 m0, %2\n\t"
                 "s_nop 0\n\t"
                 "global_load_lds_dwordx4 %1, off offset:%3\n\t"
                 "s_mov_b32 m0, %0"
                 : "=&s"(keep) : "v"(src), "s"(dst), "n"(pc * 1024) : "memory");
  };
  auto issue_advance = [&]() __attribute__((always_inline)) {
    islot = islot + 1 == R ? 0 : islot + 1;
    if (++ikt == KT) { ikt = 0; if (++isec == 3) { isec = 0; ih = ih + 1 == hb + NH ? hb : ih + 1; } }
  };

  auto run = [&](auto NT_) __attribute__((always_inline)) {
    constexpr int NT = decltype(NT_)::value;
    constexpr int NA = NT > 0 ? NT : 1;
    V8 xf[NA][NXF];

    auto load_frags = [&](int img) __attribute__((always_inline)) {
#pragma unroll
      for (int tt = 0; tt < NT; ++tt) {
        const int t0 = (2 * w + tt) * 32 + r31;
        const int t = t0 < T ? t0 : T - 1;
        const int64_t tok = (int64_t)img * T + t;
        const char* xb = static_cast<const char*>(a.xn) + (tok >> 5) * (int64_t)KC * 512 + (tok & 31) * 16 + half * 512;
#pragma unroll
        for (int i = 0; i < NXF; ++i) {
          xf[tt][i] = (QA_NT & 1) ? __builtin_nontemporal_load(reinterpret_cast<const V8*>(xb + i * 1024)) : *reinterpret_cast<const V8*>(xb + i * 1024);
        }
      }
    };
    const int nimg = (a.B - slot0 + nslots - 1) / nslots;
    const int gtotal = nimg * NH * NSH;
    int slot = 0;
    int g = 0;

    const float cexp = 0.125f * 1.44269504088896340736f;
    constexpr bool INITMASK = NTT > 2;
    f32x16 sinit;
#pragma unroll
    for (int r = 0; r < 16; ++r) sinit[r] = ((NTT - 1) * 32 + (r & 3) + 8 * (r >> 2) + 4 * (lane >> 5) >= T) ? -INFINITY : 0.f;

// ... 215 lines not shown
          if constexpr (INITMASK && kt == NTT - 1) s[kt] = sinit;
          else {
#pragma unroll
            for (int r = 0; r < 16; ++r) s[kt][r] = 0.f;
          }
#pragma unroll
          for (int ks = 0; ks < 4; ++ks) s[kt] = Op16<E>::mfma(kf[cur][ks], qf[tt][ks], s[kt]);
          __builtin_amdgcn_sched_barrier(0);
        });
        QA_STAMP_AT(5 + tt * 5)
        V8 vf[2][2];
#pragma unroll
        for (int db = 0; db < 2; ++db) vf[0][db] = *reinterpret_cast<const V8*>(vb + db * 1024);
        float mx = -INFINITY;
#pragma unroll
        for (int kt = 0; kt < NTT; ++kt) {
#pragma unroll
          for (int r = 0; r < 16; ++r) {
            if (!INITMASK) {
              const int key = kt * 32 + (r & 3) + 8 * (r >> 2) + 4 * half;
              if (key >= T) s[kt][r] = -INFINITY;
            }
            mx = fmaxf(mx, s[kt][r]);
          }
        }
        mx = fmaxf(mx, __shfl_xor(mx, 32, 64));
        f32x16 o[2];
#pragma unroll
        for (int db = 0; db < 2; ++db)
#pragma unroll
          for (int r = 0; r < 16; ++r) o[db][r] = 0.f;
        f32x16 lsum;
#pragma unroll
        for (int r = 0; r < 16; ++r) lsum[r] = 0.f;
        const V8 ones = {(E)1.f, (E)1.f, (E)1.f, (E)1.f, (E)1.f, (E)1.f, (E)1.f, (E)1.f};
        const float mxc = mx * cexp;
        __builtin_amdgcn_sched_barrier(0);
        V8 pf[2];
        float av[8], ev[8];
        auto p_part = [&](auto ST_, auto PART_) __attribute__((always_inline)) {
          constexpr int st = decltype(ST_)::value, kt = st >> 1, m = st & 1, part = decltype(PART_)::value;
          if constexpr (part == 0) {
#pragma unroll
            for (int j = 0; j < 4; ++j) av[j] = __builtin_fmaf(s[kt][8 * m + j], cexp, -mxc);
            ev[0] = __builtin_amdgcn_exp2f(av[0]); ev[1] = __builtin_amdgcn_exp2f(av[1]);
          } else if constexpr (part == 1) {
#pragma unroll
            for (int j = 4; j < 8; ++j) av[j] = __builtin_fmaf(s[kt][8 * m + j], cexp, -mxc);
            ev[2] = __builtin_amdgcn_exp2f(av[2]); ev[3] = __builtin_amdgcn_exp2f(av[3]); ev[4] = __builtin_amdgcn_exp2f(av[4]);
          } else {
            ev[5] = __builtin_amdgcn_exp2f(av[5]); ev[6] = __builtin_amdgcn_exp2f(av[6]); ev[7] = __builtin_amdgcn_exp2f(av[7]);
            const u32x4 pw = {pack2<E>(ev[0], ev[1]), pack2<E>(ev[2], ev[3]), pack2<E>(ev[4], ev[5]), pack2<E>(ev[6], ev[7])};
            pf[st & 1] = __builtin_bit_cast(V8, pw);
          }
        };
        QA_STAMP_AT(6 + tt * 5)
        qa_for<0, 3>([&](auto P_) { p_part(std::integral_constant<int, 0>{}, P_); });
        __builtin_amdgcn_sched_barrier(0);
        qa_for<0, NPV>([&](auto ST_) {
          constexpr int st = decltype(ST_)::value, cur = st & 1, nxt = cur ^ 1;
          constexpr bool more = st + 1 < NPV;
          if constexpr (more) {
#pragma unroll
            for (int db = 0; db < 2; ++db) vf[nxt][db] = *reinterpret_cast<const V8*>(vb + ((st + 1) * 2 + db) * 1024);
          }
          o[0] = Op16<E>::mfma(vf[cur][0], pf[cur], o[0]);
          __builtin_amdgcn_sched_barrier(0);
          if constexpr (more) p_part(std::integral_constant<int, st + 1>{}, std::integral_constant<int, 0>{});
          __builtin_amdgcn_sched_barrier(0);
          o[1] = Op16<E>::mfma(vf[cur][1], pf[cur], o[1]);
          __builtin_amdgcn_sched_barrier(0);
          if constexpr (more) p_part(std::integral_constant<int, st + 1>{}, std::integral_constant<int, 1>{});
          __builtin_amdgcn_sched_barrier(0);
          lsum = Op16<E>::mfma(ones, pf[cur], lsum);
          __builtin_amdgcn_sched_barrier(0);
          if constexpr (more) p_part(std::integral_constant<int, st + 1>{}, std::integral_constant<int, 2>{});
          __builtin_amdgcn_sched_barrier(0);
        });
        QA_STAMP_AT(7 + tt * 5)
        const float l = lsum[0];
        if (tq < T) {
          const float inv = 1.0f / l;
          char* ob = static_cast<char*>(a.out);
#pragma unroll
          for (int db = 0; db < 2; ++db)
#pragma unroll
            for (int p = 0; p < 2; ++p) {
              const u32x2 lo = pack4<E>(o[db][8 * p] * inv, o[db][8 * p + 1] * inv, o[db][8 * p + 2] * inv, o[db][8 * p + 3] * inv);
              const u32x2 hi = pack4<E>(o[db][8 * p + 4] * inv, o[db][8 * p + 5] * inv, o[db][8 * p + 6] * inv, o[db][8 * p + 7] * inv);
              const u32x4 v = {lo[0], lo[1], hi[0], hi[1]};
              u32x4* op = reinterpret_cast<u32x4*>(ob + blk_off(tok0 + tq, h * 8 + db * 4 + 2 * p + half, D / 8));
              if (QA_NT & 2) __builtin_nontemporal_store(v, op); else *op = v;
            }
        }
        QA_STAMP_AT(8 + tt * 5)
      });
      QA_STAMP_AT(15)
    };

    load_frags(slot0);
#pragma unroll
    for (int s0 = 0; s0 < R - 1; ++s0) {
#pragma unroll
      for (int p = 0; p < 4; ++p) issue_piece(p);
      issue_advance();
    }
    asm volatile("s_waitcnt vmcnt(%0)" ::"n"((R - 2) * 4) : "memory");
    __builtin_amdgcn_s_barrier();
    asm volatile("" ::: "memory");
#pragma unroll 1
    for (int ii = 0; ii < nimg; ++ii) {
      const int img = slot0 + ii * nslots;
      tok0 = (int64_t)img * T;
      refresh_lane();
#pragma unroll 1
      for (int i = 0; i < NH - 1; ++i) {
        const int h = hb + (h0 + i < NH ? h0 + i : h0 + i - NH);
        head(std::false_type{}, std::false_type{}, h, i, 0);
      }
      const int hl = hb + (h0 == 0 ? NH - 1 : h0 - 1);
      if (ii + 1 < nimg) head(std::false_type{}, std::true_type{}, hl, HEADS - 1, img + nslots);
      else head(std::true_type{}, std::false_type{}, hl, HEADS - 1, 0);
    }
  };

#if QA_ODD_TILE_WAVE
  if ((NTT & 1) && w == 3) run(std::integral_constant<int, 1>{});
  else
#endif
  run(std::integral_constant<int, 2>{});
}

template <typename E>
int launch_qkvattn(const QkvAttnArgs& a, hipStream_t s) {
  const int ntt = (a.T + 31) / 32;
  const int cus = device_cus();
  const int heads = a.D / 64;
  auto split_for = [&](int64_t images) {
    if (a.hsplit == 1 || a.D != 384) return 1;
    for (int c = heads; c >= 2; --c)
      if (heads % c == 0 && images * c <= cus && (a.hsplit <= 0 || c <= a.hsplit)) return c;
    return 1;
  };
  const int64_t nimg_launch = (int64_t)a.B - a.img0;
  int hs = split_for(nimg_launch);
  if (a.img0 == 0 && hs == 1 && a.B > cus && a.hsplit != 1) {
    const int tail = a.B % cus, ths = tail ? split_for(tail) : 1;
    if (ths > 1) {
      QkvAttnArgs m = a, t = a;
      m.B = a.B - tail; m.hsplit = 1;
      t.img0 = a.B - tail;
      const int rc = launch_qkvattn<E>(m, s);
      return rc ? rc : launch_qkvattn<E>(t, s);
    }
  }
  QkvAttnArgs ah = a;
  ah.hsplit = hs;
  const QkvAttnArgs& a2 = ah;
  const dim3 grid((unsigned)(hs > 1 ? nimg_launch * hs : (nimg_launch < cus ? nimg_launch : cus))), blk(256);
  const bool short_tail = a.T <= 32 * ntt - 16;
  if (a.D == 384 && ntt == 7 && a.cls_only && short_tail) { QA_REC(384, 7, 1, 13); hipLaunchKernelGGL((qkvattn_kernel<E, 384, 7, true, 13>), grid, blk, 0, s, a2); }
  else if (a.D == 384 && ntt == 7 && a.cls_only) { QA_REC(384, 7, 1, 14); hipLaunchKernelGGL((qkvattn_kernel<E, 384, 7, true>), grid, blk, 0, s, a2); }
  else if (a.D == 384 && ntt == 7 && short_tail) { QA_REC(384, 7, 0, 13); hipLaunchKernelGGL((qkvattn_kernel<E, 384, 7, false, 13>), grid, blk, 0, s, a2); }
  else if (a.D == 384 && ntt == 7) { QA_REC(384, 7, 0, 14); hipLaunchKernelGGL((qkvattn_kernel<E, 384, 7>), grid, blk, 0, s, a2); }
  else if (a.D == 384 && ntt <= 2) { QA_REC(384, 2, 0, 4); hipLaunchKernelGGL((qkvattn_kernel<E, 384, 2>), grid, blk, 0, s, a2); }
  else if (a.D == 128 && ntt == 7) { QA_REC(128, 7, 0, 14); hipLaunchKernelGGL((qkvattn_kernel<E, 128, 7>), grid, blk, 0, s, a2); }
  else if (a.D == 128 && ntt <= 2) { QA_REC(128, 2, 0, 4); hipLaunchKernelGGL((qkvattn_kernel<E, 128, 2>), grid, blk, 0, s, a2); }
  else return fail(EFFOCR_EUNSUPPORTED, "qkv_attn_fused: (embed dim, tokens) must be (128|384, <=64 or 193..224)");
  return check_launch("qkv_attn_fused");
}

}

bool qkv_attn_supported(int prec, int D, int T) {
  const int ntt = (T + 31) / 32;
  return prec != PREC_FP32 && (D == 384 || D == 128) && T >= 1 && (ntt <= 2 || ntt == 7);
}

int qkv_attn_fused(int prec, const QkvAttnArgs& a, hipStream_t s) {
  if (a.B <= 0) return EFFOCR_OK;
  if (!qkv_attn_supported(prec, a.D, a.T)) return fail(EFFOCR_EUNSUPPORTED, "qkv_attn_fused: unsupported (precision, embed dim, tokens)");
  if (a.rows_alloc % 32 || a.rows_alloc < (int64_t)a.B * a.T) return fail(EFFOCR_EINVAL, "qkv_attn_fused: rows_alloc must be a multiple of 32 >= batch * tokens");
  if ((reinterpret_cast<uintptr_t>(a.bias) & 15) != 0) return fail(EFFOCR_EINVAL, "qkv_attn_fused: the bias array must be 16-byte aligned (it reaches LDS by 16-byte DMA)");
  return prec == PREC_BF16 ? launch_qkvattn<__bf16>(a, s) : launch_qkvattn<_Float16>(a, s);
}


}

#ifdef QA_STAMP
extern "C" int effocr_debug_qa_stamps(unsigned long long* out, int n) {
  const int m = effocr::QA_STAMP_WGS * 4 * effocr::QA_STAMP_N;
  if (n < m) return -1;
  return hipMemcpyFromSymbol(out, HIP_SYMBOL(effocr::qa_stamps), (size_t)m * 8) == hipSuccess ? 0 : -2;
}
#endif
```

effocr_amd/csrc/vit_ops.hip:

```cpp
#include "common.hpp"
#include "kernels.hpp"
#include "ln.hpp"
#include <math.h>


#ifndef ATT_NT
#define ATT_NT 0
#endif
#ifndef LN_NT
#define LN_NT 1
#endif
namespace effocr {
namespace {

template <int G, int V, typename TO>
__global__ __launch_bounds__(256) void layernorm_kernel(const float* __restrict__ x, int64_t rows,
                                                        const float* __restrict__ gamma,
                                                        const float* __restrict__ beta, float eps,
                                                        TO* __restrict__ out) {
  constexpr int D = 4 * G * V;
  constexpr int RPW = 64 / G;
  const int lane = threadIdx.x & 63, sub = lane % G;
  const int64_t row = ((int64_t)blockIdx.x * 4 + (threadIdx.x >> 6)) * RPW + lane / G;
  const int64_t rc = row < rows ? row : rows - 1;
  f32x4 y[V];
  ln_row<G, V>(x + rc * D, sub, gamma, beta, eps, y);
  if (row < rows) {
#pragma unroll
    for (int i = 0; i < V; ++i) {
      TO* p = out + row * D + (sub + G * i) * 4;
      if constexpr (sizeof(TO) == 4) *reinterpret_cast<f32x4*>(p) = y[i];
      else *reinterpret_cast<u32x2*>(p) = pack4<TO>(y[i][0], y[i][1], y[i][2], y[i][3]);
    }
  }
}

struct LnReduce { const float* partial; const float* b2; float* xw; int nparts, tail_rb, add_x; };
template <int D, typename TO, bool REDUCE = false, int NP = 0>
__global__ __launch_bounds__(256) void layernorm_blocked_kernel(const float* __restrict__ x, int64_t rows,
                                                                const float* __restrict__ gamma,
                                                                const float* __restrict__ beta, float eps,
                                                                TO* __restrict__ out, LnReduce rd) {
  static_assert(sizeof(TO) == 2 && D % 32 == 0, "blocked LayerNorm writes 16-bit operands");
  constexpr int NQ = D / 32;
  __shared__ float red[2][4][32];
  const int lane = threadIdx.x & 63, tl = lane & 31, part = lane >> 5, wv = threadIdx.x >> 6;
  const int64_t rb = blockIdx.x;
  const char* xb = reinterpret_cast<const char*>(x) + rb * (D / 4) * 512 + tl * 16;
  const int c0 = wv * (D / 16) + part;
  f32x4 v[NQ];
  f32x4 gmv[REDUCE ? NQ : 1], btv[REDUCE ? NQ : 1];
  if constexpr (REDUCE) {
#pragma unroll
    for (int i = 0; i < NQ; ++i) {
      gmv[i] = *reinterpret_cast<const f32x4*>(gamma + (c0 + 2 * i) * 4);
      btv[i] = *reinterpret_cast<const f32x4*>(beta + (c0 + 2 * i) * 4);
    }
  }
  if constexpr (REDUCE) {
    const int64_t per_rb = (int64_t)(D / 4) * 32;
    const bool live = rb * 32 + tl < rows;
    f32x4 pvs[NP > 0 ? NQ : 1][NP > 0 ? NP : 1];
    if constexpr (NP > 0) {
#pragma unroll
      for (int i = 0; i < NQ; ++i)
#pragma unroll
        for (int p = 0; p < NP; ++p)
          pvs[i][p] = __builtin_nontemporal_load(reinterpret_cast<const f32x4*>(rd.partial) + ((int64_t)p * rd.tail_rb + rb) * per_rb + (int64_t)(c0 + 2 * i) * 32 + tl);
    }
#pragma unroll
    for (int i = 0; i < NQ; ++i) {
      const int c = c0 + 2 * i;
      const int64_t rem = (int64_t)c * 32 + tl;
      f32x4 acc = {0.f, 0.f, 0.f, 0.f};
      if constexpr (NP > 0) {
#pragma unroll
        for (int p = 0; p < NP; ++p)
#pragma unroll
          for (int e = 0; e < 4; ++e) acc[e] += pvs[i][p][e];
      } else
      for (int p = 0; p < rd.nparts; ++p) {
        const f32x4 pv = reinterpret_cast<const f32x4*>(rd.partial)[((int64_t)p * rd.tail_rb + rb) * per_rb + rem];
#pragma unroll
        for (int e = 0; e < 4; ++e) acc[e] += pv[e];
      }
      const f32x4 bv = *reinterpret_cast<const f32x4*>(rd.b2 + c * 4);
      f32x4 xo = {0.f, 0.f, 0.f, 0.f};
      if (rd.add_x) xo = *reinterpret_cast<const f32x4*>(xb + (size_t)c * 512);
#pragma unroll
      for (int e = 0; e < 4; ++e) v[i][e] = acc[e] + bv[e] + (rd.add_x ? xo[e] : 0.f);
      if (live) *reinterpret_cast<f32x4*>(reinterpret_cast<char*>(rd.xw) + rb * (D / 4) * 512 + tl * 16 + (size_t)c * 512) = v[i];
    }
  } else {
#pragma unroll
    for (int i = 0; i < NQ; ++i) v[i] = (LN_NT & 1) ? __builtin_nontemporal_load(reinterpret_cast<const f32x4*>(xb + (size_t)(c0 + 2 * i) * 512)) : *reinterpret_cast<const f32x4*>(xb + (size_t)(c0 + 2 * i) * 512);
  }
  float s = 0.f;
#pragma unroll
  for (int i = 0; i < NQ; ++i) s += (v[i][0] + v[i][1]) + (v[i][2] + v[i][3]);
  s += __shfl_xor(s, 32, 64);
  if (part == 0) red[0][wv][tl] = s;
  __syncthreads();
  const float mean = ((red[0][0][tl] + red[0][1][tl]) + (red[0][2][tl] + red[0][3][tl])) * (1.0f / D);
  float ss = 0.f;
#pragma unroll
  for (int i = 0; i < NQ; ++i)
#pragma unroll
    for (int e = 0; e < 4; ++e) { const float d = v[i][e] - mean; ss += d * d; }
  ss += __shfl_xor(ss, 32, 64);
  if (part == 0) red[1][wv][tl] = ss;
  __syncthreads();
  const float var = ((red[1][0][tl] + red[1][1][tl]) + (red[1][2][tl] + red[1][3][tl])) * (1.0f / D);
  const float rstd = 1.0f / sqrtf(var + eps);
  if (rb * 32 + tl >= rows) return;
  char* ob = reinterpret_cast<char*>(out) + rb * (D / 8) * 512 + tl * 16 + part * 8;
#pragma unroll
  for (int i = 0; i < NQ; ++i) {
    const int c = c0 + 2 * i;
    const f32x4 gm = REDUCE ? gmv[REDUCE ? i : 0] : *reinterpret_cast<const f32x4*>(gamma + c * 4);
    const f32x4 bt = REDUCE ? btv[REDUCE ? i : 0] : *reinterpret_cast<const f32x4*>(beta + c * 4);
    const u32x2 o = pack4<TO>((v[i][0] - mean) * rstd * gm[0] + bt[0], (v[i][1] - mean) * rstd * gm[1] + bt[1],
                              (v[i][2] - mean) * rstd * gm[2] + bt[2], (v[i][3] - mean) * rstd * gm[3] + bt[3]);
    if (LN_NT & 2) __builtin_nontemporal_store(o, reinterpret_cast<u32x2*>(ob + (size_t)(c >> 1) * 512));
    else *reinterpret_cast<u32x2*>(ob + (size_t)(c >> 1) * 512) = o;
  }
}

template <int G, int V>
__global__ __launch_bounds__(256) void cls_norm_kernel(const float* __restrict__ x, int B, int T,
                                                       const float* __restrict__ gamma,
                                                       const float* __restrict__ beta, float eps, int l2norm,
                                                       int blocked, float* __restrict__ emb, int* __restrict__ status) {
  constexpr int D = 4 * G * V;
  constexpr int RPW = 64 / G;
  const int lane = threadIdx.x & 63, sub = lane % G;
  const int img = (blockIdx.x * 4 + (threadIdx.x >> 6)) * RPW + lane / G;
  const int ic = img < B ? img : B - 1;
  f32x4 y[V], v[V];
#pragma unroll
  for (int i = 0; i < V; ++i) {
    const int chunk = sub + G * i;
    const char* p = blocked ? reinterpret_cast<const char*>(x) + blk_off((int64_t)ic * T, chunk, D / 4)
                            : reinterpret_cast<const char*>(x + (int64_t)ic * T * D + chunk * 4);
    v[i] = *reinterpret_cast<const f32x4*>(p);
  }
  ln_apply<G, V>(v, sub, gamma, beta, eps, y);
  if (l2norm) {
    float ss = 0.f;
#pragma unroll
    for (int i = 0; i < V; ++i)
#pragma unroll
      for (int e = 0; e < 4; ++e) ss += y[i][e] * y[i][e];
    const float nr = sqrtf(group_sum<G>(ss));
    const float nrm = nr < 1e-12f ? 1e-12f : nr;
#pragma unroll
    for (int i = 0; i < V; ++i)
#pragma unroll
      for (int e = 0; e < 4; ++e) y[i][e] = y[i][e] / nrm;
  }
  if (img < B) {
    bool bad = false;
#pragma unroll
    for (int i = 0; i < V; ++i) {
#pragma unroll
      for (int e = 0; e < 4; ++e) bad |= !(fabsf(y[i][e]) <= 3.0e38f);
      *reinterpret_cast<f32x4*>(emb + (int64_t)img * D + (sub + G * i) * 4) = y[i];
    }
    if (status && bad) atomicOr(status, 1);
  }
}

template <typename TO, typename TI = float>
__global__ __launch_bounds__(256) void im2col16_kernel(const TI* __restrict__ x, int B, int H, int W,
                                                       TO* __restrict__ out) {
  const int PH = H / 16, PW = W / 16;
  const int64_t total = (int64_t)B * PH * PW * 96;
  const int64_t id = (int64_t)blockIdx.x * 256 + threadIdx.x;
  if (id >= total) return;
  const int k8 = (int)(id % 96);
  const int64_t m = id / 96;
  const int px = (int)(m % PW), py = (int)((m / PW) % PH);
  const int64_t img = m / ((int64_t)PW * PH);
  const int c = k8 >> 5, ky = (k8 & 31) >> 1, kx0 = (k8 & 1) * 8;
  const TI* src = x + ((img * 3 + c) * H + (py * 16 + ky)) * (int64_t)W + px * 16 + kx0;
  TO* dst = out + m * 768 + k8 * 8;
  if constexpr (sizeof(TI) == 2) {
    static_assert(sizeof(TO) == 2, "im2col16: 16-bit crops feed 16-bit patch rows");
    *reinterpret_cast<u32x4*>(dst) = *reinterpret_cast<const u32x4*>(src);
    return;
  }
  const f32x4 a = *reinterpret_cast<const f32x4*>(reinterpret_cast<const float*>(src));
  const f32x4 b = *reinterpret_cast<const f32x4*>(reinterpret_cast<const float*>(src) + 4);
  if constexpr (sizeof(TO) == 4) {
    *reinterpret_cast<f32x4*>(dst) = a;
    *reinterpret_cast<f32x4*>(dst + 4) = b;
  } else {
    const u32x2 lo = pack4<TO>(a[0], a[1], a[2], a[3]);
    const u32x2 hi = pack4<TO>(b[0], b[1], b[2], b[3]);
    u32x4 v = {lo[0], lo[1], hi[0], hi[1]};
    *reinterpret_cast<u32x4*>(dst) = v;
  }
}

__global__ __launch_bounds__(256) void gather_cls_kernel(const float* __restrict__ x, const char* __restrict__ att, int B, int T, int D,
                                                         float* __restrict__ xc, char* __restrict__ ac) {
  const int nx = D / 4, na = D / 8;
  const int64_t id = (int64_t)blockIdx.x * 256 + threadIdx.x;
  if (id >= (int64_t)B * (nx + na)) return;
  const int img = (int)(id / (nx + na)), c = (int)(id % (nx + na));
  if (c < nx) *reinterpret_cast<f32x4*>(reinterpret_cast<char*>(xc) + blk_off(img, c, nx)) =
                  *reinterpret_cast<const f32x4*>(reinterpret_cast<const char*>(x) + blk_off((int64_t)img * T, c, nx));
  else *reinterpret_cast<u32x4*>(ac + blk_off(img, c - nx, na)) = *reinterpret_cast<const u32x4*>(att + blk_off((int64_t)img * T, c - nx, na));
}

__global__ void set_cls_kernel(const float* __restrict__ cls_pos0, float* __restrict__ x, int B, int T, int D, int blocked, int* __restrict__ status_zero) {
  const int64_t id = (int64_t)blockIdx.x * 256 + threadIdx.x;
  if (id == 0 && status_zero) *status_zero = 0;
  if (id >= (int64_t)B * D) return;
  const int d = (int)(id % D);
  const int64_t img = id / D;
  if (blocked) *reinterpret_cast<float*>(reinterpret_cast<char*>(x) + blk_off(img * T, d >> 2, D / 4) + (d & 3) * 4) = cls_pos0[d];
  else x[img * T * D + d] = cls_pos0[d];
}

// ... 198 lines not shown
#pragma unroll
    for (int c = 0; c < 16; ++c) {
      f32x4 v = {o[c * 4] * inv, o[c * 4 + 1] * inv, o[c * 4 + 2] * inv, o[c * 4 + 3] * inv};
      *reinterpret_cast<f32x4*>(orow + c * 4) = v;
    }
  }
}

template <typename TO>
int launch_ln(const float* x, int64_t rows, int D, const float* gamma, const float* beta, float eps, TO* out,
              hipStream_t s) {
  if (rows <= 0) return EFFOCR_OK;
  if (D == 384) {
    const int64_t rpb = 4 * 2;
    hipLaunchKernelGGL((layernorm_kernel<32, 3, TO>), dim3((unsigned)((rows + rpb - 1) / rpb)), dim3(256), 0, s, x, rows, gamma, beta, eps, out);
  } else if (D == 768) {
    const int64_t rpb = 4;
    hipLaunchKernelGGL((layernorm_kernel<64, 3, TO>), dim3((unsigned)((rows + rpb - 1) / rpb)), dim3(256), 0, s, x, rows, gamma, beta, eps, out);
  } else if (D == 128) {
    const int64_t rpb = 4 * 2;
    hipLaunchKernelGGL((layernorm_kernel<32, 1, TO>), dim3((unsigned)((rows + rpb - 1) / rpb)), dim3(256), 0, s, x, rows, gamma, beta, eps, out);
  } else {
    return fail(EFFOCR_EUNSUPPORTED, "layernorm: embed dim must be 128, 384 or 768");
  }
  return check_launch("layernorm");
}

template <typename TO>
int launch_ln_blocked(const float* x, int64_t rows, int D, const float* gamma, const float* beta, float eps, TO* out,
                      hipStream_t s) {
  if (rows <= 0) return EFFOCR_OK;
  const dim3 grid((unsigned)((rows + 31) / 32));
  const LnReduce none{};
  if (D == 768) hipLaunchKernelGGL((layernorm_blocked_kernel<768, TO>), grid, dim3(256), 0, s, x, rows, gamma, beta, eps, out, none);
  else if (D == 384) hipLaunchKernelGGL((layernorm_blocked_kernel<384, TO>), grid, dim3(256), 0, s, x, rows, gamma, beta, eps, out, none);
  else if (D == 128) hipLaunchKernelGGL((layernorm_blocked_kernel<128, TO>), grid, dim3(256), 0, s, x, rows, gamma, beta, eps, out, none);
  else return fail(EFFOCR_EUNSUPPORTED, "layernorm(blocked): embed dim must be 128, 384 or 768");
  return check_launch("layernorm_blocked");
}

template <typename TO, typename TI = float>
int launch_im2col(const void* x, int B, int H, int W, TO* out, hipStream_t s) {
  const int64_t total = (int64_t)B * (H / 16) * (W / 16) * 96;
  if (total <= 0) return EFFOCR_OK;
  hipLaunchKernelGGL((im2col16_kernel<TO, TI>), dim3((unsigned)((total + 255) / 256)), dim3(256), 0, s, static_cast<const TI*>(x), B, H, W, out);
  return check_launch("im2col16");
}

template <typename E, bool BLK>
int launch_attn_mfma(const E* qkv, E* out, int B, int T, int heads, hipStream_t s) {
  const int nkt = (T + 31) / 32;
  const dim3 grid((unsigned)(B * heads)), blk(256);
  switch (nkt) {
    case 1: hipLaunchKernelGGL((attn_mfma_kernel<E, 1, BLK>), grid, blk, 0, s, qkv, out, B, T, heads); break;
    case 2: hipLaunchKernelGGL((attn_mfma_kernel<E, 2, BLK>), grid, blk, 0, s, qkv, out, B, T, heads); break;
    case 7: hipLaunchKernelGGL((attn_mfma_kernel<E, 7, BLK>), grid, blk, 0, s, qkv, out, B, T, heads); break;
    default: return fail(EFFOCR_EUNSUPPORTED, "attention: token count must be <=64 or in (192,224]");
  }
  return check_launch("attention");
}

}

int gather_cls_rows_blocked(const float* x, const void* att, int B, int T, int D, float* xc, void* ac, hipStream_t s) {
  if (B <= 0) return EFFOCR_OK;
  const int64_t total = (int64_t)B * (D / 4 + D / 8);
  hipLaunchKernelGGL(gather_cls_kernel, dim3((unsigned)((total + 255) / 256)), dim3(256), 0, s, x, static_cast<const char*>(att), B, T, D, xc,
                     static_cast<char*>(ac));
  return check_launch("gather_cls");
}

int layernorm_rows(int prec_out, const float* x, int64_t rows, int D, const float* gamma, const float* beta,
                   float eps, void* out, hipStream_t s) {
  switch (prec_out) {
    case PREC_BF16: return launch_ln<__bf16>(x, rows, D, gamma, beta, eps, static_cast<__bf16*>(out), s);
    case PREC_FP16: return launch_ln<_Float16>(x, rows, D, gamma, beta, eps, static_cast<_Float16*>(out), s);
    case PREC_FP32: return launch_ln<float>(x, rows, D, gamma, beta, eps, static_cast<float*>(out), s);
  }
  return fail(EFFOCR_EINVAL, "layernorm: unknown precision");
}

template <typename TO>
int launch_reduce_ln_blocked(float* x, int64_t rows, int D, const float* partial, const float* b2, int nparts, int tail_rb, int add_x,
                             const float* gamma, const float* beta, float eps, TO* out, hipStream_t s) {
  if (rows <= 0) return EFFOCR_OK;
  const dim3 grid((unsigned)((rows + 31) / 32));
  const LnReduce rd{partial, b2, x, nparts, tail_rb, add_x};
  if (D == 384 && nparts == 6) hipLaunchKernelGGL((layernorm_blocked_kernel<384, TO, true, 6>), grid, dim3(256), 0, s, x, rows, gamma, beta, eps, out, rd);
  else if (D == 384 && nparts == 3) hipLaunchKernelGGL((layernorm_blocked_kernel<384, TO, true, 3>), grid, dim3(256), 0, s, x, rows, gamma, beta, eps, out, rd);
  else if (D == 384 && nparts == 4) hipLaunchKernelGGL((layernorm_blocked_kernel<384, TO, true, 4>), grid, dim3(256), 0, s, x, rows, gamma, beta, eps, out, rd);
  else if (D == 384 && nparts == 2) hipLaunchKernelGGL((layernorm_blocked_kernel<384, TO, true, 2>), grid, dim3(256), 0, s, x, rows, gamma, beta, eps, out, rd);
  else if (D == 384) hipLaunchKernelGGL((layernorm_blocked_kernel<384, TO, true>), grid, dim3(256), 0, s, x, rows, gamma, beta, eps, out, rd);
  else if (D == 128) hipLaunchKernelGGL((layernorm_blocked_kernel<128, TO, true>), grid, dim3(256), 0, s, x, rows, gamma, beta, eps, out, rd);
  else return fail(EFFOCR_EUNSUPPORTED, "reduce + layernorm(blocked): embed dim must be 128 or 384");
  return check_launch("reduce_layernorm_blocked");
}

int reduce_layernorm_rows_blocked(int prec_out, float* x, int64_t rows, int D, const float* partial, const float* b2, int nparts, int tail_rb,
                                  int add_x, const float* gamma, const float* beta, float eps, void* out, hipStream_t s) {
  switch (prec_out) {
    case PREC_BF16: return launch_reduce_ln_blocked<__bf16>(x, rows, D, partial, b2, nparts, tail_rb, add_x, gamma, beta, eps, static_cast<__bf16*>(out), s);
    case PREC_FP16: return launch_reduce_ln_blocked<_Float16>(x, rows, D, partial, b2, nparts, tail_rb, add_x, gamma, beta, eps, static_cast<_Float16*>(out), s);
  }
  return fail(EFFOCR_EUNSUPPORTED, "reduce + layernorm(blocked): 16-bit output only");
}

int layernorm_rows_blocked(int prec_out, const float* x, int64_t rows, int D, const float* gamma, const float* beta,
                           float eps, void* out, hipStream_t s) {
  switch (prec_out) {
    case PREC_BF16: return launch_ln_blocked<__bf16>(x, rows, D, gamma, beta, eps, static_cast<__bf16*>(out), s);
    case PREC_FP16: return launch_ln_blocked<_Float16>(x, rows, D, gamma, beta, eps, static_cast<_Float16*>(out), s);
  }
  return fail(EFFOCR_EUNSUPPORTED, "layernorm(blocked): 16-bit output only");
}

int im2col_patch16(int prec_out, const void* x, int x16, int B, int H, int W, void* out, hipStream_t s) {
  if (H % 16 || W % 16) return fail(EFFOCR_EINVAL, "im2col: image size must be a multiple of 16");
  if (x16) {
    if (prec_out == PREC_BF16) return launch_im2col<__bf16, __bf16>(x, B, H, W, static_cast<__bf16*>(out), s);
    if (prec_out == PREC_FP16) return launch_im2col<_Float16, _Float16>(x, B, H, W, static_cast<_Float16*>(out), s);
    return fail(EFFOCR_EUNSUPPORTED, "im2col: 16-bit crops need a 16-bit precision mode");
  }
  switch (prec_out) {
    case PREC_BF16: return launch_im2col<__bf16>(x, B, H, W, static_cast<__bf16*>(out), s);
    case PREC_FP16: return launch_im2col<_Float16>(x, B, H, W, static_cast<_Float16*>(out), s);
    case PREC_FP32: return launch_im2col<float>(x, B, H, W, static_cast<float*>(out), s);
  }
  return fail(EFFOCR_EINVAL, "im2col: unknown precision");
}

int set_cls_rows(const float* cls_pos0, float* x, int B, int T, int D, int blocked, int* status_zero, hipStream_t s) {
  const int64_t total = (int64_t)B * D;
  if (total <= 0) return EFFOCR_OK;
  hipLaunchKernelGGL(set_cls_kernel, dim3((unsigned)((total + 255) / 256)), dim3(256), 0, s, cls_pos0, x, B, T, D, blocked, status_zero);
  return check_launch("set_cls_rows");
}

int attention(int prec, const void* qkv, void* out, int B, int T, int heads, int blocked, hipStream_t s) {
  if (B <= 0) return EFFOCR_OK;
  if (blocked && prec == PREC_FP32) return fail(EFFOCR_EUNSUPPORTED, "attention(fp32): blocked layout not supported");
  switch (prec) {
    case PREC_BF16:
      return blocked ? launch_attn_mfma<__bf16, true>(static_cast<const __bf16*>(qkv), static_cast<__bf16*>(out), B, T, heads, s)
                     : launch_attn_mfma<__bf16, false>(static_cast<const __bf16*>(qkv), static_cast<__bf16*>(out), B, T, heads, s);
    case PREC_FP16:
      return blocked ? launch_attn_mfma<_Float16, true>(static_cast<const _Float16*>(qkv), static_cast<_Float16*>(out), B, T, heads, s)
                     : launch_attn_mfma<_Float16, false>(static_cast<const _Float16*>(qkv), static_cast<_Float16*>(out), B, T, heads, s);
    case PREC_FP32:
      if (T > ATT32_TMAX) return fail(EFFOCR_EUNSUPPORTED, "attention(fp32): more than 224 tokens");
      hipLaunchKernelGGL(attn_f32_kernel, dim3((unsigned)(B * heads)), dim3(256), 0, s,
                         static_cast<const float*>(qkv), static_cast<float*>(out), B, T, heads);
      return check_launch("attention_f32");
  }
  return fail(EFFOCR_EINVAL, "attention: unknown precision");
}

__global__ void clock_sample_kernel(unsigned long long* out) {
  const unsigned hw = __builtin_amdgcn_s_getreg((4 << 0) | (0 << 6) | (31 << 11));
  const unsigned xcc = __builtin_amdgcn_s_getreg((20 << 0) | (0 << 6) | (3 << 11)) & 7u;
  const unsigned key = xcc * 256u + ((hw >> 13) & 7u) * 32u + ((hw >> 12) & 1u) * 16u + ((hw >> 8) & 15u);
  if (threadIdx.x == 0) { out[2 * key] = __builtin_amdgcn_s_memtime(); out[2 * key + 1] = __builtin_amdgcn_s_memrealtime(); }
}
int clock_sample(unsigned long long* out, hipStream_t s) {
  hipLaunchKernelGGL(clock_sample_kernel, dim3(1024), dim3(64), 0, s, out);
  return check_launch("clock_sample");
}

int final_cls_norm(const float* x, int B, int T, int D, const float* gamma, const float* beta, float eps,
                   int l2norm, int blocked, float* emb, int* status, hipStream_t s) {
  if (B <= 0) return EFFOCR_OK;
  if (D == 384) {
    hipLaunchKernelGGL((cls_norm_kernel<32, 3>), dim3((unsigned)((B + 7) / 8)), dim3(256), 0, s, x, B, T, gamma, beta, eps, l2norm, blocked, emb, status);
  } else if (D == 768) {
    hipLaunchKernelGGL((cls_norm_kernel<64, 3>), dim3((unsigned)((B + 3) / 4)), dim3(256), 0, s, x, B, T, gamma, beta, eps, l2norm, blocked, emb, status);
  } else if (D == 128) {
    hipLaunchKernelGGL((cls_norm_kernel<32, 1>), dim3((unsigned)((B + 7) / 8)), dim3(256), 0, s, x, B, T, gamma, beta, eps, l2norm, blocked, emb, status);
  } else {
    return fail(EFFOCR_EUNSUPPORTED, "final norm: embed dim must be 128, 384 or 768");
  }
  return check_launch("final_cls_norm");
}

}
```

include/effocr_hip.h:

```cpp
#ifndef EFFOCR_HIP_H
#define EFFOCR_HIP_H

#include <stddef.h>
#include <stdint.h>

#ifdef __cplusplus
extern "C" {
#endif

#define EFFOCR_ABI_VERSION 9

enum effocr_status {
  EFFOCR_OK = 0,
  EFFOCR_EINVAL = -1,
  EFFOCR_EUNSUPPORTED = -2,
  EFFOCR_EWORKSPACE = -3,
  EFFOCR_EHIP = -4,
  EFFOCR_ESTATE = -5,
  EFFOCR_EOVERFLOW = -6
};

enum effocr_precision {
  EFFOCR_PREC_BF16 = 0,
  EFFOCR_PREC_FP16 = 1,
// ... 46 lines not shown
size_t effocr_knn_screen_flag_offset(int64_t nq, int64_t ntotal, int d, int k);
int effocr_knn_ip_topk_screened(const float* q_dev, int64_t nq, const float* xb_dev, const void* xb_bf16_dev, int64_t ntotal, int d,
                                int k, float xnorm_max, float* dist_dev, int64_t* idx_dev, void* workspace_dev,
                                size_t workspace_bytes, void* stream);
int effocr_convert_bf16(const float* src_dev, int64_t n, void* dst_dev, void* stream);
size_t effocr_bf16_blocked_bytes(int64_t n_rows, int d);
int effocr_convert_bf16_blocked(const float* src_dev, int64_t n_rows, int d, void* dst_dev, void* stream);
int effocr_knn_ip_topk_screened2(const float* q_dev, int64_t nq, const float* xb_dev, const void* xb_bf16_dev, const void* xb_bf16_blk_dev,
                                 int64_t ntotal, int d, int k, float xnorm_max, float* dist_dev, int64_t* idx_dev, void* workspace_dev,
                                 size_t workspace_bytes, void* stream);
int effocr_l2_normalize(const float* x_dev, int64_t n, int d, float* y_dev, void* stream);
int effocr_gather_rows(const float* src_dev, const int64_t* keep_rows_dev, int64_t n_keep, int d,
                       float* dst_dev, void* stream);

int effocr_crop_transform(const uint8_t* image_dev, int height, int width, int64_t row_stride,
                          const int32_t* boxes_dev, int n, int size, int antialias, const float* mean,
                          const float* std, const float* fill, float* out_dev, void* stream);

int effocr_crop_transform_batch(const uint8_t* images_dev, int n_images, int64_t image_stride, int height, int width,
                                int64_t row_stride, const int32_t* boxes_dev, int64_t n, int size, int antialias,
                                const float* mean, const float* std, const float* fill, float* out_dev, void* stream);
int effocr_crop_transform_batch_ex(const uint8_t* images_dev, int n_images, int64_t image_stride, int height, int width,
                                   int64_t row_stride, const int32_t* boxes_dev, int64_t n, int size, int antialias,
                                   const float* mean, const float* std, const float* fill, int out_dtype, void* out_dev, void* stream);

typedef struct effocr_localizer effocr_localizer_t;
int effocr_localizer_create(const char* arch, int num_classes, int in_h, int in_w, effocr_localizer_t** out);
void effocr_localizer_destroy(effocr_localizer_t* loc);
int effocr_localizer_num_params(const effocr_localizer_t* loc);
const char* effocr_localizer_param_name(const effocr_localizer_t* loc, int i);
int64_t effocr_localizer_param_numel(const effocr_localizer_t* loc, int i);
int effocr_localizer_set_param(effocr_localizer_t* loc, const char* name, const float* host, int64_t numel);
size_t effocr_localizer_weights_bytes(const effocr_localizer_t* loc);
int effocr_localizer_upload(effocr_localizer_t* loc, void* weights_dev, size_t bytes);
int effocr_localizer_set_option(effocr_localizer_t* loc, const char* name, int value);
int64_t effocr_localizer_num_predictions(const effocr_localizer_t* loc);
int effocr_localizer_num_outputs(const effocr_localizer_t* loc);
size_t effocr_localizer_workspace_bytes(const effocr_localizer_t* loc, int batch);
int effocr_localizer_forward(effocr_localizer_t* loc, const float* x_dev, int batch, float* pred_dev, void* workspace_dev,
                             size_t workspace_bytes, void* stream);
int effocr_letterbox(const uint8_t* image_dev, int height, int width, int64_t row_stride, int bgr, int out_h, int out_w, int new_h,
                     int new_w, int top, int left, float* out_dev, void* stream);
size_t effocr_nms_workspace_bytes(int n, int max_nms);
int effocr_nms(const float* pred_dev, int n, int num_classes, float conf_thres, float iou_thres, int max_det, int max_nms, float max_wh,
               int agnostic, float* out_dev, int* count_dev, void* workspace_dev, size_t workspace_bytes, void* stream);
size_t effocr_nms_batch_workspace_bytes(int n, int max_det, int max_nms);
int effocr_nms_batch(const float* pred_dev, int batch, int n, int num_classes, float conf_thres, float iou_thres, int max_det, int max_nms,
                     float max_wh, int agnostic, float* out_dev, int* count_dev, void* workspace_dev, size_t workspace_bytes, void* stream);

int effocr_parse_char_boxes(const float* rows_dev, const int* counts_dev, int lines, int max_det, int height, int width, int axis, int vertical,
                            float* sorted_dev, int* n_chars_dev, int* boxes5_dev, int* total_dev, void* stream);

enum effocr_epilogue { EFFOCR_EPI_BIAS = 0, EFFOCR_EPI_BIAS_GELU = 1, EFFOCR_EPI_BIAS_RESID = 2 };
int effocr_op_linear(int precision, int epilogue, const void* x_dev, const void* w_dev, const float* bias_dev,
                     const float* resid_dev, void* out_dev, int m, int n, int k, void* stream);
int effocr_op_ln_linear(int precision, int epilogue, const float* x_dev, const float* gamma_dev, const float* beta_dev,
                        float eps, const void* w_dev, const float* bias_dev, const float* resid_dev, void* out_dev,
                        int m, int n, int k, void* stream);
int effocr_op_layernorm(int out_precision, const float* x_dev, int64_t rows, int d, const float* gamma_dev,
                        const float* beta_dev, float eps, void* out_dev, void* stream);
int effocr_op_attention(int precision, const void* qkv_dev, void* out_dev, int batch, int tokens, int heads,
                        void* stream);

int effocr_op_linear_blocked(int precision, int epilogue, const void* x_blk_dev, const void* w_blk_dev,
                             const float* bias_dev, const float* resid_blk_dev, void* out_blk_dev, int m, int n, int k,
                             int rows_alloc, void* stream);
int effocr_op_mlp_blocked(int precision, float* x_blk_dev, const float* gamma_dev, const float* beta_dev, float eps,
                          const void* w1_blk_dev, const float* b1_dev, const void* w2_perm_dev, const float* b2_perm_dev, const float* b2_dev,
                          int m, int d, int h, int rows_alloc, void* scratch_dev, size_t scratch_bytes, void* stream);
int effocr_op_mlp_ln_blocked(int precision, float* x_blk_dev, const float* gamma_dev, const float* beta_dev, float eps,
                             const void* w1_blk_dev, const float* b1_dev, const void* w2_perm_dev, const float* b2_perm_dev, const float* b2_dev,
                             const float* gamma_next_dev, const float* beta_next_dev, void* xn_blk_dev,
                             int m, int d, int h, int rows_alloc, void* scratch_dev, size_t scratch_bytes, void* stream);
int effocr_op_proj_mlp_blocked(int precision, float* x_blk_dev, const void* a_blk_dev, const void* wp_perm_dev, const float* bp_perm_dev,
                               const float* gamma_dev, const float* beta_dev, float eps, const void* w1_blk_dev, const float* b1_dev,
                               const void* w2_perm_dev, const float* b2_perm_dev, const float* b2_dev, int m, int d, int h, int rows_alloc,
                               void* scratch_dev, size_t scratch_bytes, void* stream);

int effocr_op_qkv_attn_blocked(int precision, const void* xn_blk_dev, const void* wqkv_blk_dev, const float* bias_dev,
                               void* out_blk_dev, int batch, int tokens, int d, int rows_alloc, void* stream);
int effocr_op_layernorm_blocked(int out_precision, const float* x_blk_dev, int64_t rows, int d, const float* gamma_dev,
                                const float* beta_dev, float eps, void* out_blk_dev, void* stream);

#ifdef __cplusplus
}
#endif
#endif
```

Baseline: 104,200 glyph-crops/s.

## Write class-token rows directly into compact buffers and fuse final reduce with norm

```diff
diff --git a/effocr_amd/_lib.py b/effocr_amd/_lib.py
--- a/effocr_amd/_lib.py
+++ b/effocr_amd/_lib.py
@@ -122,6 +122,11 @@
         "effocr_op_proj_mlp_blocked": (i32, [i32, f32p, vp, vp, f32p, f32p, f32p, c.c_float, vp, f32p, vp, f32p, f32p, i32, i32, i32, i32, vp, sz, vp]),
         "effocr_op_qkv_attn_blocked": (i32, [i32, vp, vp, f32p, vp, i32, i32, i32, i32, vp]),
         "effocr_op_layernorm_blocked": (i32, [i32, f32p, i64, i32, f32p, f32p, c.c_float, vp, vp]),
+        "effocr_op_proj_mlp_blocked_ex": (i32, [i32, f32p, vp, vp, f32p, f32p, f32p, c.c_float, vp, f32p, vp, f32p, f32p, i32, i32, i32, i32, vp, sz,
+                                                f32p, f32p, vp, i32, i32, i32, i32, f32p, vp]),
+        "effocr_op_qkv_attn_blocked_ex": (i32, [i32, vp, vp, f32p, vp, vp, i32, i32, i32, i32, i32, i32, vp]),
+        "effocr_op_mlp_reduce_blocked": (i32, [f32p, f32p, f32p, i32, i32, i32, i32, vp]),
+        "effocr_op_reduce_final_norm": (i32, [f32p, f32p, i32, i32, i32, i32, f32p, f32p, c.c_float, i32, f32p, vp, vp]),
     }
     for name, (res, args) in sig.items():
         if os.environ.get("EFFOCR_HIP_LIB") and not hasattr(lib, name):
diff --git a/effocr_amd/csrc/api.hip b/effocr_amd/csrc/api.hip
--- a/effocr_amd/csrc/api.hip
+++ b/effocr_amd/csrc/api.hip
@@ -49,6 +49,7 @@
   const char* wdev = nullptr;
   int debug = 0;
   int cls_only_last = 1;
+  int cls_direct = 1;
   int mlp_stagger_min_rounds = 2;
   int mlp_tail_first = 96;
   int mlp_stagger = 2500;
@@ -611,6 +612,11 @@
   const bool qaf = blk && panel && mlpf && qkv_attn_supported(prec, D, T) && (e->use_qkvattn == 2 || (e->use_qkvattn == 1 && (e->call_size_invariant || B >= e->qa_min_batch)));
   const bool g3 = blk && e->use_gemm3 && gemm3_supported(prec, D, e->vit.mlp);
   const bool patchf = blk && e->use_patchf && patch_embed_fused_supported(prec, D);
+  const bool cd = e->cls_direct && e->cls_only_last && projf && qaf && !e->call_size_invariant;
+  const size_t Bpc = align_up((size_t)B, 128);
+  float* xc = reinterpret_cast<float*>(qkv);
+  void* ac = static_cast<char*>(qkv) + Bpc * D * 4;
+  bool direct = false;
   if (!patchf && (rc = timed(e, "im2col_patch16", 0.0, s, [&] { return im2col_patch16(prec, x, x16, B, e->img, e->img, hb, s); }))) return rc;
   int* status = reinterpret_cast<int*>(ws + w.status);
   if (!patchf && (rc = set_cls_rows(F(e->off_clspos0), xs, B, T, D, blk, nullptr, s))) return rc;
@@ -639,6 +645,7 @@
         q.xn = xn; q.Wb = wb + L.qkvw_bv; q.bias = F(L.qkvb_v); q.out = att;
         q.B = B; q.T = T; q.D = D; q.rows_alloc = (int64_t)w.rows; q.hsplit = e->qa_hsplit;
         q.cls_only = (i + 1 == e->vit.depth && e->cls_only_last && projf) ? 1 : 0;
+        if (q.cls_only && direct) q.out_cls = ac;
         const bool cls_k = q.cls_only && D == 384 && T > 192;
         const double qa_work = cls_k ? 2.0 * Md * 2.0 * Dd * Dd + 2.0 * (32.0 * B) * Dd * Dd + 4.0 * B * e->vit.heads * 32.0 * T * 64.0
                                      : 2.0 * Md * 3.0 * Dd * Dd + 4.0 * B * e->vit.heads * (double)T * T * 64.0;
@@ -666,19 +673,27 @@
         if (projf) {
           m.A = att; m.Wpp = wb + L.projw_pp; m.bp = F(L.projb_p);
           if (i + 1 == e->vit.depth && e->cls_only_last) {
-            const size_t Bp = align_up((size_t)B, 128);
-            float* xc = reinterpret_cast<float*>(qkv);
-            void* ac = static_cast<char*>(qkv) + Bp * D * 4;
-            if ((rc = timed(e, "gather_cls", 0.0, s, [&] { return gather_cls_rows_blocked(xs, att, B, T, D, xc, ac, s); }))) return rc;
-            m.x = xc; m.A = ac; m.M = B; m.rows_alloc = (int)Bp;
+            if (!direct && (rc = timed(e, "gather_cls", 0.0, s, [&] { return gather_cls_rows_blocked(xs, att, B, T, D, xc, ac, s); }))) return rc;
+            m.x = xc; m.A = ac; m.M = B; m.rows_alloc = (int)Bpc;
+            bool fin = false;
+            if (cd) {
+              m.fin_emb = emb; m.fin_gamma = F(e->off_normw); m.fin_beta = F(e->off_normb); m.fin_eps = 1e-6f; m.fin_l2 = l2; m.fin_status = status;
+              fin = mlp_fused_pair_parts(m) > 0;
+            }
             const double Bd = B;
             if ((rc = timed(e, "proj_mlp_cls", 4.0 * Bd * Hd * Dd + 2.0 * Bd * Dd * Dd, s, [&] { return mlp_fused(prec, m, s); }))) return rc;
+            if (fin) return EFFOCR_OK;
             cls_x = xc;
             continue;
           }
           if (qaf && i + 1 < e->vit.depth) {
             m.xn_out = xn; m.gamma_n = F(e->layers[i + 1].ln1w); m.beta_n = F(e->layers[i + 1].ln1b);
             xn_ready = true;
+            if (cd && i + 2 == e->vit.depth && qkv_attn_cls_kernel_for(D, T)) {
+              m.x_cls_T = T; m.x_cls_out = xc;
+              direct = mlp_fused_cls_rows_supported(m);
+              if (!direct) { m.x_cls_T = 0; m.x_cls_out = nullptr; }
+            }
           }
           if ((rc = timed(e, "proj_mlp_fused", 4.0 * Md * Hd * Dd + 2.0 * Md * Dd * Dd, s, [&] { return mlp_fused(prec, m, s); }))) return rc;
           continue;
@@ -1090,6 +1105,7 @@
   if (n == "use_patchf") { enc->use_patchf = value; return EFFOCR_OK; }
   if (n == "use_projf") { enc->use_projf = value; return EFFOCR_OK; }
   if (n == "cls_only_last") { enc->cls_only_last = value; return EFFOCR_OK; }
+  if (n == "cls_direct") { enc->cls_direct = value; return EFFOCR_OK; }
   if (n == "mlp_stagger_min_rounds") { enc->mlp_stagger_min_rounds = value < 1 ? 1 : value; return EFFOCR_OK; }
   if (n == "mlp_tail_first") { enc->mlp_tail_first = value < 0 ? 0 : value & ~7; return EFFOCR_OK; }
   if (n == "mlp_stagger") { enc->mlp_stagger = value < 0 ? 0 : value; return EFFOCR_OK; }
@@ -1443,6 +1459,52 @@
   return qkv_attn_fused(precision, q, S(stream));
 }
 
+int effocr_op_proj_mlp_blocked_ex(int precision, float* x_blk_dev, const void* a_blk_dev, const void* wp_perm_dev, const float* bp_perm_dev,
+                                  const float* gamma_dev, const float* beta_dev, float eps, const void* w1_blk_dev, const float* b1_dev,
+                                  const void* w2_perm_dev, const float* b2_perm_dev, const float* b2_dev, int m, int d, int h, int rows_alloc,
+                                  void* scratch_dev, size_t scratch_bytes, const float* gamma_next_dev, const float* beta_next_dev, void* xn_blk_dev,
+                                  int no_tail_split, int pair, int no_pair_parts, int x_cls_tokens, float* x_cls_blk_dev, void* stream) {
+  if (m > 0 && (!x_blk_dev || !a_blk_dev || !wp_perm_dev || !bp_perm_dev || !gamma_dev || !beta_dev || !w1_blk_dev || !b1_dev || !w2_perm_dev || !b2_perm_dev || !b2_dev))
+    return fail(EFFOCR_EINVAL, "op_proj_mlp_blocked_ex: NULL device pointer");
+  if (xn_blk_dev && (!gamma_next_dev || !beta_next_dev)) return fail(EFFOCR_EINVAL, "op_proj_mlp_blocked_ex: the second output needs the next norm's weight and bias");
+  if (x_cls_tokens < 0 || (x_cls_tokens > 0 && !x_cls_blk_dev)) return fail(EFFOCR_EINVAL, "op_proj_mlp_blocked_ex: x_cls_tokens > 0 needs x_cls_blk_dev");
+  MlpArgs a{};
+  a.x = x_blk_dev; a.gamma = gamma_dev; a.beta = beta_dev; a.eps = eps; a.W1b = w1_blk_dev; a.b1 = b1_dev; a.W2p = w2_perm_dev; a.b2 = b2_perm_dev;
+  a.b2_logical = b2_dev; a.A = a_blk_dev; a.Wpp = wp_perm_dev; a.bp = bp_perm_dev;
+  a.M = m; a.D = d; a.H = h; a.rows_alloc = rows_alloc; a.partial = static_cast<float*>(scratch_dev); a.partial_bytes = scratch_bytes;
+  a.xn_out = xn_blk_dev; a.gamma_n = gamma_next_dev; a.beta_n = beta_next_dev;
+  a.no_tail_split = no_tail_split ? 1 : 0; a.pair = pair; a.no_pair_parts = no_pair_parts ? 1 : 0;
+  a.x_cls_T = x_cls_tokens; a.x_cls_out = x_cls_blk_dev;
+  if (m > 0 && x_cls_tokens > 0 && !mlp_fused_cls_rows_supported(a))
+    return fail(EFFOCR_EUNSUPPORTED, "op_proj_mlp_blocked_ex: x_cls_tokens needs a call that runs as whole 128-token panels (+ split tail) with the second output");
+  return mlp_fused(precision, a, S(stream));
+}
+
+int effocr_op_qkv_attn_blocked_ex(int precision, const void* xn_blk_dev, const void* wqkv_blk_dev, const float* bias_dev, void* out_blk_dev,
+                                  void* out_cls_blk_dev, int batch, int tokens, int d, int rows_alloc, int cls_only, int hsplit, void* stream) {
+  if (batch > 0 && (!xn_blk_dev || !wqkv_blk_dev || !bias_dev || !out_blk_dev))
+    return fail(EFFOCR_EINVAL, "op_qkv_attn_blocked_ex: NULL device pointer");
+  if (batch < 0 || tokens < 1 || hsplit < 0) return fail(EFFOCR_EINVAL, "op_qkv_attn_blocked_ex: bad batch / tokens / hsplit");
+  QkvAttnArgs q{};
+  q.xn = xn_blk_dev; q.Wb = wqkv_blk_dev; q.bias = bias_dev; q.out = out_blk_dev; q.out_cls = out_cls_blk_dev;
+  q.B = batch; q.T = tokens; q.D = d; q.rows_alloc = rows_alloc; q.cls_only = cls_only ? 1 : 0; q.hsplit = hsplit;
+  return qkv_attn_fused(precision, q, S(stream));
+}
+
+int effocr_op_mlp_reduce_blocked(float* x_blk_dev, const float* partial_dev, const float* b2_dev, int nparts, int part_row_blocks, int rows, int d,
+                                 void* stream) {
+  if (rows > 0 && (!x_blk_dev || !partial_dev || !b2_dev)) return fail(EFFOCR_EINVAL, "op_mlp_reduce_blocked: NULL device pointer");
+  if (rows < 0 || nparts < 1 || d < 4 || d % 4 || (int64_t)part_row_blocks * 32 < rows) return fail(EFFOCR_EINVAL, "op_mlp_reduce_blocked: bad shape");
+  return mlp_reduce_rows(x_blk_dev, partial_dev, b2_dev, part_row_blocks, d, nparts, rows, 0, S(stream));
+}
+
+int effocr_op_reduce_final_norm(const float* partial_dev, const float* b2_dev, int nparts, int part_row_blocks, int rows, int d, const float* gamma_dev,
+                                const float* beta_dev, float eps, int l2_normalize, float* emb_dev, int* status_dev, void* stream) {
+  if (rows > 0 && (!partial_dev || !b2_dev || !gamma_dev || !beta_dev || !emb_dev)) return fail(EFFOCR_EINVAL, "op_reduce_final_norm: NULL device pointer");
+  if (rows < 0) return fail(EFFOCR_EINVAL, "op_reduce_final_norm: negative rows");
+  return reduce_final_cls_norm(partial_dev, b2_dev, nparts, part_row_blocks, nullptr, rows, d, gamma_dev, beta_dev, eps, l2_normalize ? 1 : 0, emb_dev, status_dev, S(stream));
+}
+
 int effocr_op_layernorm_blocked(int out_precision, const float* x_blk_dev, int64_t rows, int d, const float* gamma_dev,
                                 const float* beta_dev, float eps, void* out_blk_dev, void* stream) {
   if (rows > 0 && (!x_blk_dev || !gamma_dev || !beta_dev || !out_blk_dev)) return fail(EFFOCR_EINVAL, "op_layernorm_blocked: NULL device pointer");
diff --git a/effocr_amd/csrc/kernels.hpp b/effocr_amd/csrc/kernels.hpp
--- a/effocr_amd/csrc/kernels.hpp
+++ b/effocr_amd/csrc/kernels.hpp
@@ -56,9 +56,14 @@
   int tail_first;
   const void* A; const void* Wpp; const float* bp; const float* b2_logical;
   void* xn_out; const float* gamma_n; const float* beta_n;
+  int x_cls_T; float* x_cls_out;
+  float* fin_emb; const float* fin_gamma; const float* fin_beta; float fin_eps; int fin_l2; int* fin_status;
 };
 bool mlp_fused_supported(int prec, int D, int H);
 int mlp_fused(int prec, const MlpArgs& a, hipStream_t s);
+int mlp_reduce_rows(float* x, const float* partial, const float* b2, int tail_rb, int D, int nparts, int64_t M, int add_x, hipStream_t s);
+int mlp_fused_pair_parts(const MlpArgs& a);
+bool mlp_fused_cls_rows_supported(const MlpArgs& a);
 
 struct QkvAttnArgs {
   const void* xn;
@@ -66,11 +71,13 @@
   void* out;
   int B, T, D;
   int64_t rows_alloc;
+  void* out_cls;
   int cls_only;
   int img0;
   int hsplit;
 };
 bool qkv_attn_supported(int prec, int D, int T);
+bool qkv_attn_cls_kernel_for(int D, int T);
 int qkv_attn_fused(int prec, const QkvAttnArgs& a, hipStream_t s);
 
 struct PatchArgs {
@@ -107,7 +114,8 @@
 int panel_gemm(int prec, int pro, int epi, const PanelArgs& a, hipStream_t s);
 
 int reduce_layernorm_rows_blocked(int prec_out, float* x, int64_t rows, int D, const float* partial, const float* b2, int nparts, int tail_rb,
-                                  int add_x, const float* gamma, const float* beta, float eps, void* out, hipStream_t s);
+                                  int add_x, const float* gamma, const float* beta, float eps, void* out, hipStream_t s,
+                                  int cls_T = 0, int64_t row0 = 0, float* cls_out = nullptr);
 int layernorm_rows_blocked(int prec_out, const float* x, int64_t rows, int D, const float* gamma, const float* beta,
                            float eps, void* out, hipStream_t s);
 int layernorm_rows(int prec_out, const float* x, int64_t rows, int D, const float* gamma, const float* beta,
@@ -119,6 +127,8 @@
 int attention(int prec, const void* qkv, void* out, int B, int T, int heads, int blocked, hipStream_t s);
 int final_cls_norm(const float* x, int B, int T, int D, const float* gamma, const float* beta, float eps,
                    int l2norm, int blocked, float* emb, int* status, hipStream_t s);
+int reduce_final_cls_norm(const float* partial, const float* b2, int nparts, int tail_rb, const float* x_keep, int B, int D, const float* gamma,
+                          const float* beta, float eps, int l2norm, float* emb, int* status, hipStream_t s);
 
 size_t knn_workspace_bytes(int64_t B, int64_t N, int D, int k);
 int knn_ip_topk(const float* q, int64_t B, const float* xb, int64_t N, int D, int k, float* dist, int64_t* idx,
diff --git a/effocr_amd/csrc/mlp.hip b/effocr_amd/csrc/mlp.hip
--- a/effocr_amd/csrc/mlp.hip
+++ b/effocr_amd/csrc/mlp.hip
@@ -1,5 +1,6 @@
 #include "common.hpp"
 #include "kernels.hpp"
+#include "mlp_roles.hpp"
 
 namespace effocr {
 
@@ -16,6 +17,23 @@
   return (prec == PREC_BF16 || prec == PREC_FP16) && ((D == 384 && H == 1536) || (D == 128 && H == 512));
 }
 
+static MlpProjForm proj_form(const MlpArgs& a) {
+  return mlp_proj_form(a.M, a.rows_alloc, device_cus(), a.pair, a.no_split6, a.no_pair_parts, a.no_tail_split, a.partial ? a.partial_bytes : 0, a.D);
+}
+
+int mlp_fused_pair_parts(const MlpArgs& a) {
+  if (a.M <= 0 || !a.A || a.D != 384 || a.H != 1536) return 0;
+  return proj_form(a).pparts;
+}
+
+bool mlp_fused_cls_rows_supported(const MlpArgs& a) {
+  if (a.M <= 0 || !a.A || !a.xn_out) return false;
+  if (a.D == 128 && a.H == 512) return true;
+  if (a.D != 384 || a.H != 1536) return false;
+  const MlpProjForm f = proj_form(a);
+  return f.pparts == 0 && !f.pair;
+}
+
 int mlp_fused(int prec, const MlpArgs& a, hipStream_t s) {
   if (a.M <= 0) return EFFOCR_OK;
   if (!mlp_fused_supported(prec, a.D, a.H)) return fail(EFFOCR_EUNSUPPORTED, "mlp_fused: needs bf16/fp16 and (D, H) in {(384, 1536), (128, 512)}");
diff --git a/effocr_amd/csrc/mlp_bf16pair.hip b/effocr_amd/csrc/mlp_bf16pair.hip
--- a/effocr_amd/csrc/mlp_bf16pair.hip
+++ b/effocr_amd/csrc/mlp_bf16pair.hip
@@ -1,6 +1,12 @@
 #include "mlp_kernel.hpp"
 namespace effocr {
 int mlp_pair_launch_bf16(const MlpArgs& a, int tncw, unsigned grid, hipStream_t s) { return launch_mlp_pair<__bf16>(a, tncw, grid, s); }
+int mlp_reduce_rows(float* x, const float* partial, const float* b2, int tail_rb, int D, int nparts, int64_t M, int add_x, hipStream_t s) {
+  const int64_t slots4 = (int64_t)tail_rb * (D / 4) * 32;
+  if (slots4 <= 0) return EFFOCR_OK;
+  hipLaunchKernelGGL(mlp_reduce_kernel, dim3((unsigned)((slots4 + 255) / 256)), dim3(256), 0, s, x, partial, b2, (int64_t)0, tail_rb, D, nparts, M, add_x);
+  return check_launch("mlp_reduce");
+}
 }
 #ifdef MLP_STAMP
 extern "C" int effocr_debug_mlp_pair_stamps(unsigned long long* out, int n) {
diff --git a/effocr_amd/csrc/mlp_kernel.hpp b/effocr_amd/csrc/mlp_kernel.hpp
--- a/effocr_amd/csrc/mlp_kernel.hpp
+++ b/effocr_amd/csrc/mlp_kernel.hpp
@@ -953,6 +953,12 @@
     });
   } else if (!PAIR && !PARTIAL && rb * 32 + r31 < a.M) {
     char* xr = reinterpret_cast<char*>(a.x) + rb * (D / 4) * 512 + r31 * 16;
+    bool xst = true;
+    if (a.x_cls_T > 0) {
+      const int row = (int)(rb * 32 + r31), ci = row / a.x_cls_T;
+      xst = row == ci * a.x_cls_T;
+      xr = reinterpret_cast<char*>(a.x_cls_out) + (size_t)(ci >> 5) * (D / 4) * 512 + (ci & 31) * 16;
+    }
     float sm = 0.f;
     sfor<0, OT>([&](auto T_) {
       constexpr int t = decltype(T_)::value;
@@ -960,7 +966,7 @@
       for (int q = 0; q < 4; ++q) {
         const f32x4 o = {acc2[t][4 * q], acc2[t][4 * q + 1], acc2[t][4 * q + 2], acc2[t][4 * q + 3]};
         sm += (o[0] + o[1]) + (o[2] + o[3]);
-        st_act<4>(reinterpret_cast<f32x4*>(xr + (size_t)cq(t, q) * 512), o);
+        if (xst) st_act<4>(reinterpret_cast<f32x4*>(xr + (size_t)cq(t, q) * 512), o);
       }
     });
     MLP_STAMP_AT(9)
@@ -1100,6 +1106,7 @@
   for (const void* q : {(const void*)a.b1, (const void*)a.b2, (const void*)a.gamma, (const void*)a.beta, (const void*)a.bp, (const void*)a.gamma_n, (const void*)a.beta_n})
     if ((reinterpret_cast<uintptr_t>(q) & 15) != 0) return fail(EFFOCR_EINVAL, "mlp_fused: bias / LayerNorm parameter arrays must be 16-byte aligned (they reach LDS by 16-byte DMA)");
   const int npanels = (a.M + MLP_PT - 1) / MLP_PT;
+  if (a.x_cls_T > 0 && (!a.x_cls_out || !PROJ)) return fail(EFFOCR_EINVAL, "mlp_fused: x_cls_T needs x_cls_out and the projection form");
   const int tail_first_opt = a.tail_first;
   a.tail_first = 0;
   if (a.D == 128 && a.H == 512) {
@@ -1111,14 +1118,16 @@
   const int slots = device_cus();
   if constexpr (PROJ) {
     const int np64 = (a.M + 63) / 64;
-    const bool fits = np64 <= slots && a.rows_alloc >= np64 * 64;
-    const int pparts = (np64 * 6 <= slots && !a.no_split6) ? 6 : np64 * 3 <= slots ? 3 : 2;
-    if (fits && (pparts > 2 || np64 * 16 <= slots * 7) && a.pair == 0 && !a.no_pair_parts && !a.no_tail_split && a.partial &&
-        a.partial_bytes >= (size_t)pparts * np64 * 64 * a.D * sizeof(float)) {
+    const MlpProjForm form = mlp_proj_form(a.M, a.rows_alloc, slots, a.pair, a.no_split6, a.no_pair_parts, a.no_tail_split, a.partial ? a.partial_bytes : 0, a.D);
+    const int pparts = form.pparts;
+    if ((pparts > 0 || form.pair) && a.x_cls_T > 0) return fail(EFFOCR_EINVAL, "mlp_fused: x_cls_T needs a call of whole 128-token panels (mlp_fused_cls_rows_supported)");
+    if (pparts > 0) {
       a.panel0 = 0; a.main_wgs = 0; a.stagger_wgs = 0; a.tail_rb = np64 * 2;
       const int prec = std::is_same<E, __bf16>::value ? PREC_BF16 : PREC_FP16;
       int rc = prec == PREC_BF16 ? mlp_pair_launch_bf16(a, 12 / pparts, (unsigned)(np64 * pparts), s) : mlp_pair_launch_f16(a, 12 / pparts, (unsigned)(np64 * pparts), s);
       if (rc) return rc;
+      if (a.fin_emb && !a.xn_out)
+        return reduce_final_cls_norm(a.partial, a.b2_logical, pparts, a.tail_rb, nullptr, a.M, a.D, a.fin_gamma, a.fin_beta, a.fin_eps, a.fin_l2, a.fin_emb, a.fin_status, s);
       if (a.xn_out && MLP_FUSED_REDUCE_LN)
         return reduce_layernorm_rows_blocked(prec, a.x, (int64_t)a.M, a.D, a.partial, a.b2_logical, pparts, a.tail_rb, 0, a.gamma_n, a.beta_n, a.eps, a.xn_out, s);
       const int64_t slots4 = (int64_t)a.tail_rb * (a.D / 4) * 32;
@@ -1127,7 +1136,7 @@
       if (rc || !a.xn_out) return rc;
       return layernorm_rows_blocked(prec, a.x, (int64_t)a.M, a.D, a.gamma_n, a.beta_n, a.eps, a.xn_out, s);
     }
-    if (fits && (a.pair > 0 || (a.pair == 0 && !a.no_tail_split && npanels * 11 > slots * 2))) {
+    if (form.pair) {
       a.panel0 = 0; a.main_wgs = np64; a.stagger_wgs = 0; a.tail_rb = 0;
       return std::is_same<E, __bf16>::value ? mlp_pair_launch_bf16(a, 0, (unsigned)np64, s) : mlp_pair_launch_f16(a, 0, (unsigned)np64, s);
     }
@@ -1156,8 +1165,9 @@
   if (a.xn_out && MLP_FUSED_REDUCE_LN) {
     return reduce_layernorm_rows_blocked(prec, reinterpret_cast<float*>(reinterpret_cast<char*>(a.x) + rb0 * (a.D / 4) * 512), (int64_t)a.M - rb0 * 32, a.D,
                                          a.partial, a.b2_logical, split, a.tail_rb, PROJ ? 0 : 1, a.gamma_n, a.beta_n, a.eps,
-                                         static_cast<char*>(a.xn_out) + rb0 * (a.D / 8) * 512, s);
-  }
+                                         static_cast<char*>(a.xn_out) + rb0 * (a.D / 8) * 512, s, a.x_cls_T, rb0 * 32, a.x_cls_out);
+  }
+  if (a.x_cls_T > 0) return fail(EFFOCR_EINVAL, "mlp_fused: x_cls_T with a split tail needs the second output (the reduction + LayerNorm launch stores the class-token rows)");
   const int64_t slots4 = (int64_t)a.tail_rb * (a.D / 4) * 32;
   hipLaunchKernelGGL(mlp_reduce_kernel, dim3((unsigned)((slots4 + 255) / 256)), dim3(256), 0, s, a.x, a.partial, a.b2_logical,
                      rb0, a.tail_rb, a.D, split, (int64_t)a.M, PROJ ? 0 : 1);
diff --git a/effocr_amd/csrc/mlp_roles.hpp b/effocr_amd/csrc/mlp_roles.hpp
--- a/effocr_amd/csrc/mlp_roles.hpp
+++ b/effocr_amd/csrc/mlp_roles.hpp
@@ -28,4 +28,17 @@
   return mlp_role_clamped(bid, main_panels, tf > 0 ? slots : 0, tf);
 }
 
+struct MlpProjForm { int pparts; bool pair; };
+constexpr MlpProjForm mlp_proj_form(int M, int rows_alloc, int slots, int pair, int no_split6, int no_pair_parts, int no_tail_split,
+                                    unsigned long long partial_bytes, int D) {
+  const int npanels = (M + 127) / 128, np64 = (M + 63) / 64;
+  const bool fits = np64 <= slots && rows_alloc >= np64 * 64;
+  const int pparts = (np64 * 6 <= slots && !no_split6) ? 6 : np64 * 3 <= slots ? 3 : 2;
+  if (fits && (pparts > 2 || np64 * 16 <= slots * 7) && pair == 0 && !no_pair_parts && !no_tail_split &&
+      partial_bytes >= (unsigned long long)pparts * np64 * 64 * D * sizeof(float))
+    return MlpProjForm{pparts, false};
+  if (fits && (pair > 0 || (pair == 0 && !no_tail_split && npanels * 11 > slots * 2))) return MlpProjForm{0, true};
+  return MlpProjForm{0, false};
 }
+
+}
diff --git a/effocr_amd/csrc/qkvattn.hip b/effocr_amd/csrc/qkvattn.hip
--- a/effocr_amd/csrc/qkvattn.hip
+++ b/effocr_amd/csrc/qkvattn.hip
@@ -75,6 +75,7 @@
   QA_STAMP_AT(14)
   const int T = a.T;
   int64_t tok0 = 0;
+  int img_cur = 0;
   const int HS = a.hsplit > 1 ? a.hsplit : 1, NH = HEADS / HS;
   const int grp = (int)blockIdx.x % HS, slot0 = a.img0 + (int)blockIdx.x / HS, nslots = (int)gridDim.x / HS;
   const int hb = grp * NH;
@@ -456,6 +457,11 @@
         if (tq < T) {
           const float inv = 1.0f / l;
           char* ob = static_cast<char*>(a.out);
+          int64_t orow = tok0 + tq;
+          bool ost = true;
+          if constexpr (CLS) {
+            if (a.out_cls != nullptr) { ob = static_cast<char*>(a.out_cls); orow = img_cur; ost = tq == 0; }
+          }
 #pragma unroll
           for (int db = 0; db < 2; ++db)
 #pragma unroll
@@ -463,8 +469,8 @@
               const u32x2 lo = pack4<E>(o[db][8 * p] * inv, o[db][8 * p + 1] * inv, o[db][8 * p + 2] * inv, o[db][8 * p + 3] * inv);
               const u32x2 hi = pack4<E>(o[db][8 * p + 4] * inv, o[db][8 * p + 5] * inv, o[db][8 * p + 6] * inv, o[db][8 * p + 7] * inv);
               const u32x4 v = {lo[0], lo[1], hi[0], hi[1]};
-              u32x4* op = reinterpret_cast<u32x4*>(ob + blk_off(tok0 + tq, h * 8 + db * 4 + 2 * p + half, D / 8));
-              if (QA_NT & 2) __builtin_nontemporal_store(v, op); else *op = v;
+              u32x4* op = reinterpret_cast<u32x4*>(ob + blk_off(orow, h * 8 + db * 4 + 2 * p + half, D / 8));
+              if (!CLS || ost) { if (QA_NT & 2) __builtin_nontemporal_store(v, op); else *op = v; }
             }
         }
         QA_STAMP_AT(8 + tt * 5)
@@ -486,6 +492,7 @@
     for (int ii = 0; ii < nimg; ++ii) {
       const int img = slot0 + ii * nslots;
       tok0 = (int64_t)img * T;
+      img_cur = img;
       refresh_lane();
 #pragma unroll 1
       for (int i = 0; i < NH - 1; ++i) {
@@ -546,6 +553,8 @@
 
 }
 
+bool qkv_attn_cls_kernel_for(int D, int T) { return D == 384 && (T + 31) / 32 == 7; }
+
 bool qkv_attn_supported(int prec, int D, int T) {
   const int ntt = (T + 31) / 32;
   return prec != PREC_FP32 && (D == 384 || D == 128) && T >= 1 && (ntt <= 2 || ntt == 7);
@@ -556,6 +565,7 @@
   if (!qkv_attn_supported(prec, a.D, a.T)) return fail(EFFOCR_EUNSUPPORTED, "qkv_attn_fused: unsupported (precision, embed dim, tokens)");
   if (a.rows_alloc % 32 || a.rows_alloc < (int64_t)a.B * a.T) return fail(EFFOCR_EINVAL, "qkv_attn_fused: rows_alloc must be a multiple of 32 >= batch * tokens");
   if ((reinterpret_cast<uintptr_t>(a.bias) & 15) != 0) return fail(EFFOCR_EINVAL, "qkv_attn_fused: the bias array must be 16-byte aligned (it reaches LDS by 16-byte DMA)");
+  if (a.out_cls && !(a.cls_only && qkv_attn_cls_kernel_for(a.D, a.T))) return fail(EFFOCR_EINVAL, "qkv_attn_fused: out_cls needs cls_only on a shape with the class-token kernel");
   return prec == PREC_BF16 ? launch_qkvattn<__bf16>(a, s) : launch_qkvattn<_Float16>(a, s);
 }
 
diff --git a/effocr_amd/csrc/vit_ops.hip b/effocr_amd/csrc/vit_ops.hip
--- a/effocr_amd/csrc/vit_ops.hip
+++ b/effocr_amd/csrc/vit_ops.hip
@@ -35,7 +35,7 @@
   }
 }
 
-struct LnReduce { const float* partial; const float* b2; float* xw; int nparts, tail_rb, add_x; };
+struct LnReduce { const float* partial; const float* b2; float* xw; int nparts, tail_rb, add_x; int cls_T; int64_t row0; float* cls_out; };
 template <int D, typename TO, bool REDUCE = false, int NP = 0>
 __global__ __launch_bounds__(256) void layernorm_blocked_kernel(const float* __restrict__ x, int64_t rows,
                                                                 const float* __restrict__ gamma,
@@ -59,7 +59,13 @@
   }
   if constexpr (REDUCE) {
     const int64_t per_rb = (int64_t)(D / 4) * 32;
-    const bool live = rb * 32 + tl < rows;
+    bool live = rb * 32 + tl < rows;
+    char* xwr = reinterpret_cast<char*>(rd.xw) + rb * (D / 4) * 512 + tl * 16;
+    if (rd.cls_T > 0) {
+      const int64_t grow = rd.row0 + rb * 32 + tl, img = grow / rd.cls_T;
+      live = live && grow == img * rd.cls_T;
+      xwr = reinterpret_cast<char*>(rd.cls_out) + (img >> 5) * (D / 4) * 512 + (img & 31) * 16;
+    }
     f32x4 pvs[NP > 0 ? NQ : 1][NP > 0 ? NP : 1];
     if constexpr (NP > 0) {
 #pragma unroll
@@ -89,7 +95,7 @@
       if (rd.add_x) xo = *reinterpret_cast<const f32x4*>(xb + (size_t)c * 512);
 #pragma unroll
       for (int e = 0; e < 4; ++e) v[i][e] = acc[e] + bv[e] + (rd.add_x ? xo[e] : 0.f);
-      if (live) *reinterpret_cast<f32x4*>(reinterpret_cast<char*>(rd.xw) + rb * (D / 4) * 512 + tl * 16 + (size_t)c * 512) = v[i];
+      if (live) *reinterpret_cast<f32x4*>(xwr + (size_t)c * 512) = v[i];
     }
   } else {
 #pragma unroll
@@ -126,11 +132,12 @@
   }
 }
 
-template <int G, int V>
+struct ClsReduce { const float* partial; const float* b2; int nparts, tail_rb, add_x; };
+template <int G, int V, bool RED = false>
 __global__ __launch_bounds__(256) void cls_norm_kernel(const float* __restrict__ x, int B, int T,
                                                        const float* __restrict__ gamma,
                                                        const float* __restrict__ beta, float eps, int l2norm,
-                                                       int blocked, float* __restrict__ emb, int* __restrict__ status) {
+                                                       int blocked, float* __restrict__ emb, int* __restrict__ status, ClsReduce rd) {
   constexpr int D = 4 * G * V;
   constexpr int RPW = 64 / G;
   const int lane = threadIdx.x & 63, sub = lane % G;
@@ -140,6 +147,21 @@
 #pragma unroll
   for (int i = 0; i < V; ++i) {
     const int chunk = sub + G * i;
+    if constexpr (RED) {
+      const int64_t per_rb = (int64_t)(D / 4) * 32, rbl = ic >> 5, rem = (int64_t)chunk * 32 + (ic & 31);
+      f32x4 xo = {0.f, 0.f, 0.f, 0.f};
+      if (rd.add_x) xo = reinterpret_cast<const f32x4*>(x)[rbl * per_rb + rem];
+      const f32x4 bv = *reinterpret_cast<const f32x4*>(rd.b2 + chunk * 4);
+      f32x4 acc = {0.f, 0.f, 0.f, 0.f};
+      for (int p = 0; p < rd.nparts; ++p) {
+        const f32x4 pv = reinterpret_cast<const f32x4*>(rd.partial)[((int64_t)p * rd.tail_rb + rbl) * per_rb + rem];
+#pragma unroll
+        for (int e = 0; e < 4; ++e) acc[e] += pv[e];
+      }
+#pragma unroll
+      for (int e = 0; e < 4; ++e) v[i][e] = acc[e] + bv[e] + (rd.add_x ? xo[e] : 0.f);
+      continue;
+    }
     const char* p = blocked ? reinterpret_cast<const char*>(x) + blk_off((int64_t)ic * T, chunk, D / 4)
                             : reinterpret_cast<const char*>(x + (int64_t)ic * T * D + chunk * 4);
     v[i] = *reinterpret_cast<const f32x4*>(p);
@@ -504,10 +526,11 @@
 
 template <typename TO>
 int launch_reduce_ln_blocked(float* x, int64_t rows, int D, const float* partial, const float* b2, int nparts, int tail_rb, int add_x,
-                             const float* gamma, const float* beta, float eps, TO* out, hipStream_t s) {
+                             const float* gamma, const float* beta, float eps, TO* out, hipStream_t s, int cls_T, int64_t row0, float* cls_out) {
   if (rows <= 0) return EFFOCR_OK;
+  if (cls_T > 0 && !cls_out) return fail(EFFOCR_EINVAL, "reduce + layernorm(blocked): class-token rows need their compact buffer");
   const dim3 grid((unsigned)((rows + 31) / 32));
-  const LnReduce rd{partial, b2, x, nparts, tail_rb, add_x};
+  const LnReduce rd{partial, b2, x, nparts, tail_rb, add_x, cls_T > 0 ? cls_T : 0, row0, cls_out};
   if (D == 384 && nparts == 6) hipLaunchKernelGGL((layernorm_blocked_kernel<384, TO, true, 6>), grid, dim3(256), 0, s, x, rows, gamma, beta, eps, out, rd);
   else if (D == 384 && nparts == 3) hipLaunchKernelGGL((layernorm_blocked_kernel<384, TO, true, 3>), grid, dim3(256), 0, s, x, rows, gamma, beta, eps, out, rd);
   else if (D == 384 && nparts == 4) hipLaunchKernelGGL((layernorm_blocked_kernel<384, TO, true, 4>), grid, dim3(256), 0, s, x, rows, gamma, beta, eps, out, rd);
@@ -519,10 +542,11 @@
 }
 
 int reduce_layernorm_rows_blocked(int prec_out, float* x, int64_t rows, int D, const float* partial, const float* b2, int nparts, int tail_rb,
-                                  int add_x, const float* gamma, const float* beta, float eps, void* out, hipStream_t s) {
+                                  int add_x, const float* gamma, const float* beta, float eps, void* out, hipStream_t s, int cls_T, int64_t row0,
+                                  float* cls_out) {
   switch (prec_out) {
-    case PREC_BF16: return launch_reduce_ln_blocked<__bf16>(x, rows, D, partial, b2, nparts, tail_rb, add_x, gamma, beta, eps, static_cast<__bf16*>(out), s);
-    case PREC_FP16: return launch_reduce_ln_blocked<_Float16>(x, rows, D, partial, b2, nparts, tail_rb, add_x, gamma, beta, eps, static_cast<_Float16*>(out), s);
+    case PREC_BF16: return launch_reduce_ln_blocked<__bf16>(x, rows, D, partial, b2, nparts, tail_rb, add_x, gamma, beta, eps, static_cast<__bf16*>(out), s, cls_T, row0, cls_out);
+    case PREC_FP16: return launch_reduce_ln_blocked<_Float16>(x, rows, D, partial, b2, nparts, tail_rb, add_x, gamma, beta, eps, static_cast<_Float16*>(out), s, cls_T, row0, cls_out);
   }
   return fail(EFFOCR_EUNSUPPORTED, "reduce + layernorm(blocked): 16-bit output only");
 }
@@ -592,15 +616,25 @@
                    int l2norm, int blocked, float* emb, int* status, hipStream_t s) {
   if (B <= 0) return EFFOCR_OK;
   if (D == 384) {
-    hipLaunchKernelGGL((cls_norm_kernel<32, 3>), dim3((unsigned)((B + 7) / 8)), dim3(256), 0, s, x, B, T, gamma, beta, eps, l2norm, blocked, emb, status);
+    hipLaunchKernelGGL((cls_norm_kernel<32, 3>), dim3((unsigned)((B + 7) / 8)), dim3(256), 0, s, x, B, T, gamma, beta, eps, l2norm, blocked, emb, status, ClsReduce{});
   } else if (D == 768) {
-    hipLaunchKernelGGL((cls_norm_kernel<64, 3>), dim3((unsigned)((B + 3) / 4)), dim3(256), 0, s, x, B, T, gamma, beta, eps, l2norm, blocked, emb, status);
+    hipLaunchKernelGGL((cls_norm_kernel<64, 3>), dim3((unsigned)((B + 3) / 4)), dim3(256), 0, s, x, B, T, gamma, beta, eps, l2norm, blocked, emb, status, ClsReduce{});
   } else if (D == 128) {
-    hipLaunchKernelGGL((cls_norm_kernel<32, 1>), dim3((unsigned)((B + 7) / 8)), dim3(256), 0, s, x, B, T, gamma, beta, eps, l2norm, blocked, emb, status);
+    hipLaunchKernelGGL((cls_norm_kernel<32, 1>), dim3((unsigned)((B + 7) / 8)), dim3(256), 0, s, x, B, T, gamma, beta, eps, l2norm, blocked, emb, status, ClsReduce{});
   } else {
     return fail(EFFOCR_EUNSUPPORTED, "final norm: embed dim must be 128, 384 or 768");
   }
   return check_launch("final_cls_norm");
 }
 
-}
+int reduce_final_cls_norm(const float* partial, const float* b2, int nparts, int tail_rb, const float* x_keep, int B, int D, const float* gamma,
+                          const float* beta, float eps, int l2norm, float* emb, int* status, hipStream_t s) {
+  if (B <= 0) return EFFOCR_OK;
+  if (D != 384) return fail(EFFOCR_EUNSUPPORTED, "reduce + final norm: embed dim must be 384");
+  if (nparts < 1 || (int64_t)tail_rb * 32 < B) return fail(EFFOCR_EINVAL, "reduce + final norm: the partial rows do not cover the batch");
+  const ClsReduce rd{partial, b2, nparts, tail_rb, x_keep ? 1 : 0};
+  hipLaunchKernelGGL((cls_norm_kernel<32, 3, true>), dim3((unsigned)((B + 7) / 8)), dim3(256), 0, s, x_keep, B, 1, gamma, beta, eps, l2norm, 1, emb, status, rd);
+  return check_launch("reduce_final_cls_norm");
+}
+
+}
diff --git a/include/effocr_hip.h b/include/effocr_hip.h
--- a/include/effocr_hip.h
+++ b/include/effocr_hip.h
@@ -152,6 +152,18 @@
 int effocr_op_layernorm_blocked(int out_precision, const float* x_blk_dev, int64_t rows, int d, const float* gamma_dev,
                                 const float* beta_dev, float eps, void* out_blk_dev, void* stream);
 
+int effocr_op_proj_mlp_blocked_ex(int precision, float* x_blk_dev, const void* a_blk_dev, const void* wp_perm_dev, const float* bp_perm_dev,
+                                  const float* gamma_dev, const float* beta_dev, float eps, const void* w1_blk_dev, const float* b1_dev,
+                                  const void* w2_perm_dev, const float* b2_perm_dev, const float* b2_dev, int m, int d, int h, int rows_alloc,
+                                  void* scratch_dev, size_t scratch_bytes, const float* gamma_next_dev, const float* beta_next_dev, void* xn_blk_dev,
+                                  int no_tail_split, int pair, int no_pair_parts, int x_cls_tokens, float* x_cls_blk_dev, void* stream);
+int effocr_op_qkv_attn_blocked_ex(int precision, const void* xn_blk_dev, const void* wqkv_blk_dev, const float* bias_dev, void* out_blk_dev,
+                                  void* out_cls_blk_dev, int batch, int tokens, int d, int rows_alloc, int cls_only, int hsplit, void* stream);
+int effocr_op_mlp_reduce_blocked(float* x_blk_dev, const float* partial_dev, const float* b2_dev, int nparts, int part_row_blocks, int rows, int d,
+                                 void* stream);
+int effocr_op_reduce_final_norm(const float* partial_dev, const float* b2_dev, int nparts, int part_row_blocks, int rows, int d, const float* gamma_dev,
+                                const float* beta_dev, float eps, int l2_normalize, float* emb_dev, int* status_dev, void* stream);
+
 #ifdef __cplusplus
 }
 #endif
```

Result: no change. 104,400 glyph-crops/s (median of 6 runs) (+0.2%).
